# sinhvt3421/scann--material

Measured on AMD Instinct MI355X. Metric: QM9 molecules/s forward, higher is better.
Workload: dtype f32 (projections: split-fp16 hi/lo operands, 3 v_mfma_f32_32x32x16_f16 per product, fp32 accumulate; everything else fp32)

## Files before the change

include/scann_hip.h:

```cpp
#ifndef SCANN_HIP_H
#define SCANN_HIP_H

#include <stdint.h>

#ifdef __cplusplus
extern "C" {
#endif

#define SCANN_ABI_VERSION 1

typedef enum scann_status {
  SCANN_OK = 0,
  SCANN_ERR_INVALID = -1,
  SCANN_ERR_UNSUPPORTED = -2,
  SCANN_ERR_NO_DEVICE = -3,
  SCANN_ERR_HIP = -4,
  SCANN_ERR_WEIGHTS = -5,
  SCANN_ERR_OOM = -6,
  SCANN_ERR_RANGE = -7
} scann_status;

typedef struct scann_config {
  int32_t n_atoms;
  int32_t embedding_dim;
  int32_t local_dim;
  int32_t num_head;
  int32_t n_attention;
  int32_t global_dim;
  int32_t dense_out;
  int32_t n_gauss;
  float gaussian_d;
  int32_t g_update;
  int32_t use_attn_norm;
  int32_t use_ga_norm;
  int32_t use_ring;
  int32_t feature_cgcnn;
  int32_t relu_out;
} scann_config_t;

typedef struct scann_tensor_desc {
  const char* name;
  int64_t offset;
  int64_t numel;
} scann_tensor_desc_t;

typedef struct scann_batch {
  int32_t n_struct;
  int32_t n_atom;
  int32_t n_edge;
  const int32_t* atomic;
  const int32_t* mol_offset;
  const int32_t* edge_offset;
  const int32_t* edge_col;
  const float* edge_dist;
  const float* edge_weight;
  const float* ring;
  const float* cgcnn;
} scann_batch_t;

typedef struct scann_handle scann_handle_t;
typedef struct scann_dbatch scann_dbatch_t;

typedef struct scann_profile {
  float ms_basis;
  float ms_atom;
  float ms_edge;
  float ms_readout;
  float ms_total;
  int32_t n_edge_launch;
  int32_t n_atom_launch;
  int32_t reserved;
} scann_profile_t;

int scann_abi_version(void);
int scann_device_count(void);

int scann_create(const scann_config_t* cfg, int device_id, scann_handle_t** out);
void scann_destroy(scann_handle_t* h);
const char* scann_last_error(const scann_handle_t* h);

int scann_weight_count(const scann_handle_t* h);
int scann_weight_name(const scann_handle_t* h, int index, const char** name, int64_t* rows, int64_t* cols);

int scann_load_weights(scann_handle_t* h, const float* blob, const scann_tensor_desc_t* manifest, int n);

int scann_forward(scann_handle_t* h, const scann_batch_t* batch, float* y_out, float* ga_attn_out);

int scann_forward_padded(scann_handle_t* h, int32_t B, int32_t M, int32_t N, const int32_t* atomic,
                         const uint8_t* atom_mask, const int32_t* neighbors, const uint8_t* neighbor_mask,
                         const float* neighbor_weight, const float* neighbor_distance, float* y_out, float* ga_out);

int scann_batch_upload(scann_handle_t* h, const scann_batch_t* batch, scann_dbatch_t** out);
int scann_upload_padded(scann_handle_t* h, int32_t B, int32_t M, int32_t N, const int32_t* atomic, const void* atom_mask,
                        int32_t atom_mask_size, const int32_t* neighbors, const void* neighbor_mask, int32_t neighbor_mask_size,
                        const float* neighbor_weight, const float* neighbor_distance, scann_dbatch_t** out, int32_t* n_atom_out,
                        int32_t* n_edge_out);
int scann_batch_read_csr(scann_handle_t* h, scann_dbatch_t* db, int32_t* atomic, int32_t* mol_offset, int32_t* edge_offset,
                         int32_t* edge_col, float* edge_dist, float* edge_weight);
void scann_batch_free(scann_handle_t* h, scann_dbatch_t* db);
void scann_batch_release(scann_handle_t* h, scann_dbatch_t* db);
int scann_forward_resident(scann_handle_t* h, scann_dbatch_t* db, int stream_slot);
int scann_batch_download(scann_handle_t* h, scann_dbatch_t* db, float* y_out, float* ga_attn_out);
int scann_batch_info(scann_handle_t* h, const scann_dbatch_t* db, int32_t* out8);
int scann_sync(scann_handle_t* h);
int scann_device_memory(scann_handle_t* h, int64_t* free_bytes, int64_t* total_bytes);
int64_t scann_exact_reruns(const scann_handle_t* h);
int scann_weights_exact(const scann_handle_t* h);
int scann_num_streams(const scann_handle_t* h);

#define SCANN_OUT_LOCAL_ATTENTION 0
#define SCANN_OUT_AFTER_LC 1
#define SCANN_OUT_BF_PROPERTY 2
int scann_set_outputs(scann_handle_t* h, uint64_t attn_layers, int32_t flags);
int64_t scann_output_read(scann_handle_t* h, scann_dbatch_t* db, int32_t what, int32_t layer, float* out, int64_t cap);

int scann_forward_profile(scann_handle_t* h, scann_dbatch_t* db, scann_profile_t* prof);

int scann_edge_timing(scann_handle_t* h, int every);
int scann_edge_timing_read(scann_handle_t* h, double* avg_us, int64_t* n_launches, double* avg_edges);

int scann_set_debug(scann_handle_t* h, int on);
int scann_debug_read(scann_handle_t* h, scann_dbatch_t* db, int what, int layer, float* out);
int64_t scann_train_debug_read(scann_handle_t* h, scann_dbatch_t* db, const char* name, float* out, int64_t cap);

int scann_debug_stamps(scann_handle_t* h, scann_dbatch_t* db, uint64_t* out, int max_tiles);

int64_t scann_param_count(const scann_handle_t* h);
int scann_train_begin(scann_handle_t* h);
int scann_train_forward(scann_handle_t* h, scann_dbatch_t* db, const float* targets, float dropout, uint64_t seed, double* sse_out);
int scann_train_backward(scann_handle_t* h, scann_dbatch_t* db, double sse_global, int64_t count_global);
int scann_set_attention_dropout(scann_handle_t* h, float p);
int scann_set_deterministic(scann_handle_t* h, int on);
int scann_zero_grads(scann_handle_t* h);
int scann_allreduce_grads(scann_handle_t* h);
int scann_allreduce_sse(scann_handle_t* h, double* sse, int64_t* count);
int scann_adam_step(scann_handle_t* h, float lr_t, float beta1, float beta2, float eps, float l2);
int scann_train_step(scann_handle_t* h, scann_dbatch_t* db, const float* targets, float dropout, uint64_t seed, float lr_t, float beta1,
                     float beta2, float eps, float l2, double* sse_out, int64_t* count_out);
int scann_train_step_begin(scann_handle_t* h, scann_dbatch_t* db, const float* targets, float dropout, uint64_t seed, float lr_t, float beta1,
                           float beta2, float eps, float l2);
int scann_train_step_end(scann_handle_t* h, double* sse_out, int64_t* count_out, double* abs_err_out );
int scann_get_grads(scann_handle_t* h, float* out);
int scann_get_weights(scann_handle_t* h, float* out);

int scann_input_grads(scann_handle_t* h, scann_dbatch_t* db, float* y, float* d_distance, float* d_weight,
                      float* d_ring, float* d_cgcnn);

int scann_predict_mc(scann_handle_t* h, scann_dbatch_t* db, int32_t n_samples, uint64_t seed, const uint64_t* keys, float p_drop, float p_attn,
                     float* y_mean, float* y_std, float* ga_mean, float* ga_std, float* y_samples);
double scann_mc_drop_scale(uint64_t seed, int32_t t, uint64_t key, uint32_t tag, uint64_t idx, float p);

#define SCANN_ABLATE_LEAVE_ONE_OUT 0
#define SCANN_ABLATE_DELETION 1
#define SCANN_ABLATE_INSERTION 2
#define SCANN_ABLATE_MAX_ATOMS 960
int scann_ablate_pooling(scann_handle_t* h, scann_dbatch_t* db, int32_t mode, float* y, float* ga, float* y_abl, int32_t* order);

int scann_shapley(scann_handle_t* h, scann_dbatch_t* db, int32_t n_perm, uint64_t seed, const uint64_t* keys, const int32_t* perms_in,
                  float* y, float* ga, double* shapley, double* stderr_out, double* baseline, double* full, float* values, int32_t* perms_out);
int scann_shapley_profile(scann_handle_t* h, scann_dbatch_t* db, int32_t n_perm, uint64_t seed, const uint64_t* keys, float* ms);
void scann_shapley_permutation(uint64_t seed, uint64_t key, int32_t p, int32_t n, int32_t* out);
int scann_shapley_reduce_host(const float* values, const int32_t* perms, const int32_t* mol_offset, int32_t n_struct, int32_t n_perm,
                              const double* baseline, double* shapley, double* stderr_out, double* full);

#define SCANN_ROLLOUT_MAX_ATOMS 960
int64_t scann_rollout_floats(scann_handle_t* h, const scann_dbatch_t* db);
int scann_attention_rollout(scann_handle_t* h, scann_dbatch_t* db, float residual, int32_t head, int32_t depth, float* y, float* ga,
                            float* attribution, float* rollout);

#define SCANN_KNN_MAX_K 32
typedef struct scann_index scann_index_t;
int scann_index_create(scann_handle_t* h, int32_t dim, scann_index_t** out);
void scann_index_free(scann_handle_t* h, scann_index_t* idx);
int64_t scann_index_size(const scann_index_t* idx);
int scann_index_add(scann_handle_t* h, scann_index_t* idx, const float* rows, int64_t n, const int64_t* ids, const int32_t* atoms);
int scann_index_read(scann_handle_t* h, scann_index_t* idx, int64_t first, int64_t n, float* rows, int64_t* ids, int32_t* atoms);
int scann_index_query(scann_handle_t* h, scann_index_t* idx, const float* q, int64_t nq, const int64_t* query_ids, int32_t k, float* dist2,
                      int64_t* ids, int32_t* atoms, int32_t* pos);
int scann_index_add_batch(scann_handle_t* h, scann_index_t* idx, scann_dbatch_t* db, int32_t level, const int64_t* ids);
// ... 110 lines not shown
                       int64_t* sums);
int scann_peaks_host(const float* rows, int64_t n, int64_t dim, float gamma, int64_t* sums, int32_t* parent, float* delta2);

#define SCANN_MST_MAX_ROWS 262144
int scann_index_mst(scann_handle_t* h, scann_index_t* pool, const float* core2 , int64_t* n_edges,
                    int32_t* a , int32_t* b, float* w, int32_t* rounds );
int scann_mst_host(const float* rows, int64_t n, int64_t dim, const float* core2, int64_t* n_edges, int32_t* a, int32_t* b, float* w);
int scann_mst_last_rounds(int32_t cap, int32_t* components, double* seconds, int64_t* skipped, int64_t* tiles);

int scann_index_silhouette(scann_handle_t* h, scann_index_t* pool, const int32_t* labels , int32_t C,
                           const int32_t* qpos , int64_t nq, int32_t squared, int32_t shift,
                           int64_t* counts , double* a , double* b , int32_t* other ,
                           int64_t* sums );
int scann_silhouette_host(const float* rows, int64_t n, int64_t dim, const int32_t* labels, int32_t C, const int32_t* qpos, int64_t nq,
                          int32_t squared, int32_t shift, int32_t threads, int64_t* counts, double* a, double* b, int32_t* other,
                          int64_t* sums);

#define SCANN_RANKS_MAX_PROBES 32
#define SCANN_RANKS_SLICE 262144
int scann_index_ranks(scann_handle_t* h, scann_index_t* pool,
                      const int32_t* qpos , int64_t nq,
                      const int32_t* probe , int32_t m,
                      int32_t* rank , float* dist2 );
int scann_ranks_host(const float* rows, int64_t n, int64_t dim, const int32_t* qpos, int64_t nq, const int32_t* probe, int32_t m,
                     int32_t threads, int32_t* rank, float* dist2);

int scann_index_partition(scann_handle_t* h, scann_index_t* idx, int32_t cells, int32_t max_iter, int64_t* info );
int scann_index_partition_args(const scann_index_t* idx, int32_t* cells, int32_t* max_iter);
int scann_index_cells_read(scann_handle_t* h, scann_index_t* idx, int64_t* info , float* centres, int32_t* perm, int32_t* first_tile,
                           float* lo, float* hi);
int scann_index_search_stats(const scann_index_t* idx, int64_t* out );
int scann_index_query_rows(scann_handle_t* h, scann_index_t* idx, int64_t first, int64_t n, int32_t k, float* dist2, int64_t* ids,
                           int32_t* atoms, int32_t* pos);
int64_t scann_cells_capacity(int64_t n, int32_t cells);
int scann_cells_host(const float* rows, int64_t n, int64_t dim, int32_t cells, int32_t max_iter, int64_t* info, float* centres, int32_t* perm,
                     int32_t* first_tile, float* lo, float* hi);
double scann_cell_bound(float D, float lo, float hi);

#define SCANN_WITHIN_MAX_CAP ((int64_t)1 << 30)
int scann_index_within(scann_handle_t* h, scann_index_t* idx, const float* q, int64_t nq, const int64_t* query_ids, float radius2, int64_t cap,
                       int64_t* counts , int64_t* total, float* dist2, int32_t* pos, int64_t* ids, int32_t* atoms );
int scann_index_within_rows(scann_handle_t* h, scann_index_t* idx, int64_t first, int64_t n, int32_t upper, float radius2, int64_t cap,
                            int64_t* counts, int64_t* total, float* dist2, int32_t* pos, int64_t* ids, int32_t* atoms);
int scann_index_within_batch(scann_handle_t* h, scann_index_t* idx, scann_dbatch_t* db, int32_t level, const int64_t* query_ids, float radius2,
                             int64_t cap, float* y, float* ga, int64_t* counts, int64_t* total, float* dist2, int32_t* pos, int64_t* ids,
                             int32_t* atoms);
int scann_within_host(const float* rows, int64_t n, int64_t dim, const int64_t* row_ids, const float* q, int64_t nq, const int64_t* query_ids,
                      const int32_t* query_pos, int32_t upper, float radius2, int64_t cap, int64_t* counts, int64_t* total, float* dist2,
                      int32_t* pos);

int scann_comm_unique_id(char* out128);
int scann_comm_init(scann_handle_t* h, const char* id128, int rank, int world);
int scann_comm_ranks(scann_handle_t* h);
int scann_broadcast_weights(scann_handle_t* h, int root);

int scann_models_load(scann_handle_t* h, int32_t n_models, const float* const* blobs, const scann_tensor_desc_t* const* manifests,
                      const int32_t* n_tensors, const int32_t* relu_out);
int scann_models_count(const scann_handle_t* h);
int scann_forward_models(scann_handle_t* h, scann_dbatch_t* db, int stream_slot);
int scann_models_download(scann_handle_t* h, scann_dbatch_t* db, float* y, float* ga);

const char* scann_pack_last_error(void);
int scann_pack_padded(int32_t B, int32_t M, int32_t N, const int32_t* atomic, const float* cgcnn,
                      const uint8_t* atom_mask, const int32_t* neighbors, const uint8_t* neighbor_mask,
                      const float* neighbor_weight, const float* neighbor_distance, const float* ring,
                      int32_t* out_atomic, float* out_cgcnn, float* out_ring, int32_t* out_mol_offset,
                      int32_t* out_edge_offset, int32_t* out_edge_col, float* out_edge_dist,
                      float* out_edge_weight, int32_t* out_row_of, int32_t* n_atom, int32_t* n_edge);
int scann_slice_count(const int64_t* ds_mol_offset, const int64_t* ds_edge_offset, const int64_t* sel, int32_t n_sel,
                      int64_t n_struct_total, int64_t* n_atom, int64_t* n_edge);
int scann_slice_batch(const int64_t* ds_mol_offset, const int64_t* ds_edge_offset, const int32_t* ds_atomic,
                      const float* ds_ring, const int32_t* ds_edge_local, const float* ds_edge_dist,
                      const float* ds_edge_weight, const int64_t* sel, int32_t n_sel, int64_t n_struct_total,
                      int32_t* out_atomic, float* out_ring, int32_t* out_mol_offset, int32_t* out_edge_offset,
                      int32_t* out_edge_col, float* out_edge_dist, float* out_edge_weight);
int scann_count_padded(int32_t B, int32_t M, int32_t N, const void* atom_mask, int32_t atom_mask_size, const void* neighbor_mask,
                       int32_t neighbor_mask_size, int32_t* out_mol_offset, int32_t* out_edge_offset, int32_t* out_row_of,
                       int32_t* n_atom, int32_t* n_edge);
int scann_host_copy(void* dst, const void* src, int64_t bytes);
int scann_plan_tiles(const scann_batch_t* batch, int32_t tile_rows, int32_t tile_atoms, int32_t allow_chunks, int32_t cap,
                     int32_t* tiles_out, int32_t* part_out, int32_t* n_tiles, int32_t* n_slots);
int scann_plan_tiles_filled(const scann_batch_t* batch, int32_t tile_rows, int32_t tile_atoms, int32_t cap, int32_t* atom_row_out,
                            int32_t* tile_offset_out, int32_t* tiles_out, int32_t* n_tiles);
int scann_batch_tile_plan(scann_handle_t* h, const scann_dbatch_t* batch, int32_t* out2);

#ifdef __cplusplus
}
#endif
#endif
```

scann--material_amd/csrc/scann_batch.cpp:

```cpp
#include "scann_runtime.h"

namespace {

struct PaddedSrc {
  int32_t M, N;
  const int32_t *atomic, *neighbors;
  const void* neighbor_mask;
  int32_t mask_size;
  const float *weight, *dist;
  const int32_t* row_of;
  const int32_t *d_atomic = nullptr, *d_neighbors = nullptr;
  const void* d_mask = nullptr;
  const float *d_weight = nullptr, *d_dist = nullptr;
};

}

static inline void par_memcpy(void* dst, const void* src, size_t bytes) { (void)scann_host_copy(dst, src, (int64_t)bytes); }

static int upload_impl(scann_handle_t* h, const scann_batch_t* b, scann_dbatch_t** out, bool scratch, const PaddedSrc* pad = nullptr) {
  if (!h || !b || !out) return fail(h, SCANN_ERR_INVALID, "scann_batch_upload: null argument");
  *out = nullptr;
  const int32_t B = b->n_struct, A = b->n_atom, E = b->n_edge;
  if (B <= 0 || A <= 0 || E < 0) return fail(h, SCANN_ERR_INVALID, "scann_batch_upload: empty batch");
  if (!b->mol_offset || !b->edge_offset ||
      (!pad && ((!b->atomic && !h->cfg.feature_cgcnn) || (E > 0 && (!b->edge_col || !b->edge_dist || !b->edge_weight)))))
    return fail(h, SCANN_ERR_INVALID, "scann_batch_upload: null array");
  if (pad && (h->cfg.feature_cgcnn || h->cfg.use_ring || h->t_master))
    return fail(h, SCANN_ERR_UNSUPPORTED, "scann_upload_padded: atomic feature without ring, inference handles (a training handle needs the edges on the host)");
  if (b->mol_offset[0] != 0 || b->mol_offset[B] != A || b->edge_offset[0] != 0 || b->edge_offset[A] != E)
    return fail(h, SCANN_ERR_INVALID, "scann_batch_upload: offsets do not cover the batch");
  int32_t max_atoms = 0;
  for (int s = 0; s < B; ++s) {
    const int32_t n = b->mol_offset[s + 1] - b->mol_offset[s];
    if (n <= 0) return fail(h, SCANN_ERR_INVALID, "scann_batch_upload: structure without atoms");
    max_atoms = std::max(max_atoms, n);
  }
  if ((size_t)max_atoms * 5 * sizeof(float) > 60000) return fail(h, SCANN_ERR_UNSUPPORTED, "scann_batch_upload: structure too large");
  if ((uint64_t)std::max(A, E) * D * 4 >= (1ull << 32))
    return fail(h, SCANN_ERR_UNSUPPORTED, "scann_batch_upload: more than 8,388,607 atoms or edges in one batch; split it");
  if (pad) {
  } else if (!h->cfg.feature_cgcnn) {
    for (int a = 0; a < A; ++a)
      if (b->atomic[a] < 0 || b->atomic[a] >= h->cfg.n_atoms)
        return fail(h, SCANN_ERR_INVALID, "scann_batch_upload: atomic number outside the embedding table (n_atoms)");
  } else if (!b->cgcnn) {
    return fail(h, SCANN_ERR_INVALID, "scann_batch_upload: feature=cgcnn needs batch.cgcnn [n_atom,92]");
  }
  if (h->cfg.use_ring && !b->ring) return fail(h, SCANN_ERR_INVALID, "scann_batch_upload: use_ring needs batch.ring [n_atom,2]");
  std::vector<int32_t> edge_row;
  std::vector<EdgeTile> tiles;
  std::vector<int32_t> tile_part, big_tab;
  int32_t n_slot = 0, max_degree = 0;
  int tile_rows = TE_MAX;
  {
    std::string err;
    const bool small = E > 0 && E <= 32 * 1024;
    int r = plan_tiles(b->mol_offset, B, b->edge_offset, pad ? nullptr : b->edge_col, A, E, small ? 32 : TE_MAX, h->tile_atoms, true, tiles,
                       tile_part, big_tab, edge_row, &tile_rows, &max_degree, &n_slot, err, false);
    if (r) return fail(h, r, "scann_batch_upload: " + err);
    if (small && max_degree > 32) {
      r = plan_tiles(b->mol_offset, B, b->edge_offset, pad ? nullptr : b->edge_col, A, E, TE_MAX, h->tile_atoms, true, tiles, tile_part, big_tab, edge_row,
                     &tile_rows, &max_degree, &n_slot, err, false);
      if (r) return fail(h, r, "scann_batch_upload: " + err);
    }
  }
  const int32_t n_big = (int32_t)big_tab.size() / 3;
  const bool tile_side = h->cfg.g_update && !h->generic && E > 0;
  const size_t n_ftile = tiles.size();
  HIPCHK(h, hipSetDevice(h->device));
  scann_dbatch* db = nullptr;
  if (scratch) {
    if (!h->sc_db) h->sc_db = new scann_dbatch();
    db = h->sc_db;
    if (db->dbg_c || db->stamps) (void)hipStreamSynchronize(h->streams[0]);
    cached_free(db->dbg_c);
    cached_free(db->dbg_g);
    cached_free(db->dbg_ctx);
    cached_free(db->fill_block);
    if (db->stamps) (void)hipFree(db->stamps);
    char* const gen_ws = db->gen_ws;
    const size_t gen_ws_bytes = db->gen_ws_bytes;
    char* const out_block = db->out_block;
    const size_t out_cap = db->out_cap;
    char* const mc_ws = db->mc_ws;
    const size_t mc_bytes = db->mc_bytes;
    char* const set_ws = db->set_ws;
    const size_t set_bytes = db->set_bytes;
    *db = scann_dbatch();
    db->set_ws = set_ws; db->set_bytes = set_bytes;
    db->gen_ws = gen_ws; db->gen_ws_bytes = gen_ws_bytes;
    db->out_block = out_block; db->out_cap = out_cap;
    db->mc_ws = mc_ws; db->mc_bytes = mc_bytes;
    db->owns_arena = false;
  } else {
    db = new scann_dbatch();
  }
  db->n_struct = B; db->n_atom = A; db->n_edge = E; db->n_tile = (int32_t)tiles.size(); db->max_atoms = max_atoms; db->tile_rows = tile_rows; db->max_degree = max_degree; db->tile_atoms = h->tile_atoms; db->n_big = n_big; db->n_slot = n_slot;
  size_t off = 0;
  auto take = [&](size_t bytes) { const size_t o = off; off = align_up(off + bytes); return o; };
  const size_t o_atomic = take((size_t)A * 4), o_mol = take((size_t)(B + 1) * 4), o_eoff = take((size_t)(A + 1) * 4);
  const size_t o_col = take((size_t)E * 4), o_row = take((size_t)E * 4), o_dist = take((size_t)E * 4), o_wgt = take((size_t)E * 4);
  const size_t o_tiles = take(tiles.size() * sizeof(EdgeTile));
  const size_t o_tpart = take(n_big ? tiles.size() * 4 : 0), o_big = take((size_t)n_big * 3 * 4);
  const size_t o_inoff = take((size_t)(A + 1) * 4), o_inedge = take((size_t)E * 4);
  const size_t o_ring = take(h->cfg.use_ring ? (size_t)A * 2 * 4 : 0), o_cg = take(h->cfg.feature_cgcnn ? (size_t)A * 92 * 4 : 0);
  const size_t BM = pad ? (size_t)B * pad->M : 0, BMN = pad ? BM * pad->N : 0;
  const bool pre = pad && pad->d_atomic;
  const size_t o_prow = take(BM * 4), o_pat = take(pre ? 0 : BM * 4), o_pnbr = take(pre ? 0 : BMN * 4);
  const size_t o_pmask = take(pad && !pre ? BMN * pad->mask_size : 0), o_pw = take(pre ? 0 : BMN * 4), o_pd = take(pre ? 0 : BMN * 4);
  const size_t in_bytes = off;
  const size_t rowA = (size_t)A * D * 4, rowE = (size_t)std::max(E, 1) * D * 4;
  const size_t o_geom = take(h->cfg.g_update ? rowE + D * 4 : 0);
  const size_t o_gd = take(h->cfg.g_update ? 0 : (size_t)std::max(E, 1) * NG * 4);
  const size_t o_c0 = take((h->cfg.use_ring || h->cfg.feature_cgcnn) ? rowA : 0);
  const size_t o_c = take(rowA), o_ctx = take(rowA), o_P1 = take(rowA), o_P3 = take(rowA), o_q = take(rowA);
  const size_t o_gq = take(rowA), o_gk = take(rowA), o_ga = take((size_t)A * 4), o_y = take((size_t)B * 4);
  const size_t o_pflag = take(pad ? 4 : 0);
  const size_t o_pbuf = take((size_t)n_slot * 3 * D * 4);
  const size_t slot_bytes = tile_side ? n_ftile * TQ * 4 : 0;
  const size_t o_tatom = take(slot_bytes), o_te0 = take(slot_bytes), o_tsp = take(h->cfg.feature_cgcnn ? 0 : slot_bytes);
  hipError_t e = hipSuccess;
  scann_handle::Stage* stage = nullptr;
  char* img_ptr = nullptr;
  if (scratch) {
    if (off > h->sc_cap) {
      if (h->sc_arena) { (void)hipStreamSynchronize(h->streams[0]); (void)hipFree(h->sc_arena); h->sc_arena = nullptr; h->sc_cap = 0; }
      const size_t want = off + off / 2;
      e = hipMalloc((void**)&h->sc_arena, want);
      if (e == hipSuccess) h->sc_cap = want;
    }
    if (e == hipSuccess && in_bytes > h->sc_host_cap) {
      if (h->sc_host) { (void)hipStreamSynchronize(h->streams[0]); (void)hipHostFree(h->sc_host); h->sc_host = nullptr; h->sc_host_cap = 0; }
      const size_t want = in_bytes + in_bytes / 2;
      e = hipHostMalloc((void**)&h->sc_host, want, hipHostMallocDefault);
      if (e == hipSuccess) h->sc_host_cap = want;
    }
    db->arena = h->sc_arena;
    img_ptr = h->sc_host;
  } else {
    e = cached_malloc((void**)&db->arena, off);
    if (e == hipSuccess && !h->copy_stream) e = hipStreamCreateWithFlags(&h->copy_stream, hipStreamNonBlocking);
    if (e == hipSuccess) {
      stage = &h->stage[h->stage_next++ % scann_handle::N_STAGE];
      if (stage->used) (void)hipEventSynchronize(stage->ev);
      if (!stage->ev) e = hipEventCreateWithFlags(&stage->ev, hipEventDisableTiming);
      if (e == hipSuccess && in_bytes > stage->cap) {
        if (stage->p) (void)hipHostFree(stage->p);
        stage->p = nullptr; stage->cap = 0;
        const size_t want = in_bytes + in_bytes / 4;
        e = hipHostMalloc((void**)&stage->p, want, hipHostMallocDefault);
        if (e == hipSuccess) stage->cap = want;
      }
      img_ptr = stage->p;
    }
  }
  if (e != hipSuccess) {
    if (!scratch) {
      if (db->arena) cached_free(db->arena);
      delete db;
    }
    return fail(h, e == hipErrorOutOfMemory ? SCANN_ERR_OOM : SCANN_ERR_HIP, std::string("hipMalloc(batch arena): ") + hipGetErrorString(e));
  }
  struct ImgView { char* p; char* data() const { return p; } } img{img_ptr};
  if (b->atomic && !pad) memcpy(img.data() + o_atomic, b->atomic, (size_t)A * 4);
  if (pad) memcpy(img.data() + o_prow, pad->row_of, BM * 4);
  if (pad && !pre) {
    memcpy(img.data() + o_pat, pad->atomic, BM * 4);
    par_memcpy(img.data() + o_pnbr, pad->neighbors, BMN * 4);
    par_memcpy(img.data() + o_pmask, pad->neighbor_mask, BMN * pad->mask_size);
    par_memcpy(img.data() + o_pw, pad->weight, BMN * 4);
    par_memcpy(img.data() + o_pd, pad->dist, BMN * 4);
  }
  if (h->cfg.use_ring) memcpy(img.data() + o_ring, b->ring, (size_t)A * 2 * 4);
  if (h->cfg.feature_cgcnn) memcpy(img.data() + o_cg, b->cgcnn, (size_t)A * 92 * 4);
  memcpy(img.data() + o_mol, b->mol_offset, (size_t)(B + 1) * 4);
  memcpy(img.data() + o_eoff, b->edge_offset, (size_t)(A + 1) * 4);
  if (E > 0 && !pad) {
    memcpy(img.data() + o_col, b->edge_col, (size_t)E * 4);
    memcpy(img.data() + o_dist, b->edge_dist, (size_t)E * 4);
    memcpy(img.data() + o_wgt, b->edge_weight, (size_t)E * 4);
  }
  memcpy(img.data() + o_tiles, tiles.data(), tiles.size() * sizeof(EdgeTile));
  const bool want_rev = h->t_master != nullptr;
  if (want_rev) {
    int32_t* in_off = reinterpret_cast<int32_t*>(img.data() + o_inoff);
    int32_t* in_edge = reinterpret_cast<int32_t*>(img.data() + o_inedge);
    memset(in_off, 0, (size_t)(A + 1) * 4);
    for (int e = 0; e < E; ++e) ++in_off[b->edge_col[e] + 1];
    for (int a = 0; a < A; ++a) in_off[a + 1] += in_off[a];
    std::vector<int32_t> fill(in_off, in_off + A);
    for (int e = 0; e < E; ++e) in_edge[fill[b->edge_col[e]]++] = e;
  }
  if (n_big) {
    memcpy(img.data() + o_tpart, tile_part.data(), tiles.size() * 4);
    memcpy(img.data() + o_big, big_tab.data(), (size_t)n_big * 3 * 4);
  }
  int32_t* const d_eoff = (int32_t*)(db->arena + o_eoff);
  int32_t* const d_erow = (int32_t*)(db->arena + o_row);
  PackPaddedArgs pa{};
  if (pad) {
    char* a0 = db->arena;
    pa.B = B; pa.M = pad->M; pa.N = pad->N; pa.n_species = h->cfg.n_atoms;
    pa.row_of = (const int32_t*)(a0 + o_prow); pa.edge_offset = d_eoff; pa.atomic = pre ? pad->d_atomic : (const int32_t*)(a0 + o_pat);
    pa.neighbors = pre ? pad->d_neighbors : (const int32_t*)(a0 + o_pnbr); pa.neighbor_mask = pre ? pad->d_mask : a0 + o_pmask;
    pa.mask_size = pad->mask_size;
    pa.weight = pre ? pad->d_weight : (const float*)(a0 + o_pw); pa.dist = pre ? pad->d_dist : (const float*)(a0 + o_pd);
    pa.out_atomic = (int32_t*)(a0 + o_atomic); pa.out_col = (int32_t*)(a0 + o_col);
    pa.out_dist = (float*)(a0 + o_dist); pa.out_weight = (float*)(a0 + o_wgt);
    pa.flag = (int32_t*)(a0 + o_pflag);
  }
  TileOrderArgs ta{};
  if (tile_side) {
    char* a0 = db->arena;
    ta.tiles = (const EdgeTile*)(a0 + o_tiles); ta.n_tile = (int32_t)n_ftile; ta.n_atom = A;
    ta.edge_offset = d_eoff; ta.atomic = h->cfg.feature_cgcnn ? nullptr : (const int32_t*)(a0 + o_atomic);
    ta.tile_atom = (int32_t*)(a0 + o_tatom); ta.tile_edge0 = (int32_t*)(a0 + o_te0); ta.tile_species = (int32_t*)(a0 + o_tsp);
  }
  if (scratch) {
    if (e == hipSuccess) e = hipMemcpyAsync(db->arena, img.data(), in_bytes, hipMemcpyHostToDevice, h->streams[0]);
    if (e == hipSuccess && (E > 0 || pad)) launch_edge_row(d_eoff, E > 0 ? A : 0, d_erow, h->streams[0], pad ? pa.flag : nullptr);
    if (e == hipSuccess && pad) launch_pack_padded(pa, h->streams[0]);
    if (e == hipSuccess && tile_side) launch_tile_order(ta, h->streams[0]);
  } else {
    if (e == hipSuccess) e = hipMemcpyAsync(db->arena, img.data(), in_bytes, hipMemcpyHostToDevice, h->copy_stream);
    if (e == hipSuccess && (E > 0 || pad)) launch_edge_row(d_eoff, E > 0 ? A : 0, d_erow, h->copy_stream, pad ? pa.flag : nullptr);
    if (e == hipSuccess && pad) launch_pack_padded(pa, h->copy_stream);
    if (e == hipSuccess && tile_side) launch_tile_order(ta, h->copy_stream);
    if (e == hipSuccess) e = hipEventRecord(stage->ev, h->copy_stream);
    if (e == hipSuccess) stage->used = true;
    if (e == hipSuccess) e = hipEventCreateWithFlags(&db->upload_ev, hipEventDisableTiming);
    if (e == hipSuccess) e = hipEventRecord(db->upload_ev, h->copy_stream);
  }
  if (e != hipSuccess) {
    if (!scratch) {
      (void)hipStreamSynchronize(h->copy_stream);
      if (db->upload_ev) (void)hipEventDestroy(db->upload_ev);
      cached_free(db->arena);
      delete db;
    }
    return fail(h, SCANN_ERR_HIP, std::string("hipMemcpy(batch inputs): ") + hipGetErrorString(e));
  }
  char* a0 = db->arena;
  db->atomic = (int32_t*)(a0 + o_atomic); db->mol_offset = (int32_t*)(a0 + o_mol); db->edge_offset = (int32_t*)(a0 + o_eoff);
  db->edge_col = (int32_t*)(a0 + o_col); db->edge_row = (int32_t*)(a0 + o_row);
  db->dist = (float*)(a0 + o_dist); db->weight = (float*)(a0 + o_wgt); db->tiles = (EdgeTile*)(a0 + o_tiles);
  db->in_off = (int32_t*)(a0 + o_inoff); db->in_edge = (int32_t*)(a0 + o_inedge);
  db->has_rev = want_rev;
  db->n_ftile = (int32_t)n_ftile;
  db->f_tiles = db->tiles; db->t_offset = db->edge_offset; db->t_col = db->edge_col; db->t_row = db->edge_row;
  db->t_dist = db->dist; db->t_weight = db->weight;
  if (tile_side) {
    db->tile_atom = (int32_t*)(a0 + o_tatom); db->tile_edge0 = (int32_t*)(a0 + o_te0);
    db->tile_species = h->cfg.feature_cgcnn ? nullptr : (int32_t*)(a0 + o_tsp);
  }
  db->ring = (float*)(a0 + o_ring); db->cgcnn = (float*)(a0 + o_cg); db->c0 = (float*)(a0 + o_c0);
  db->geom = (float*)(a0 + o_geom); db->gd = (float*)(a0 + o_gd);
  db->c = (float*)(a0 + o_c); db->ctx = (float*)(a0 + o_ctx); db->P1 = (float*)(a0 + o_P1); db->P3 = (float*)(a0 + o_P3);
  db->q = (float*)(a0 + o_q); db->gq = (float*)(a0 + o_gq); db->gk = (float*)(a0 + o_gk);
  db->ga = (float*)(a0 + o_ga); db->y = (float*)(a0 + o_y);
  db->pack_flag = pad ? (int32_t*)(a0 + o_pflag) : nullptr;
  if (n_big) {
    db->tile_part = (int32_t*)(a0 + o_tpart); db->big_tab = (int32_t*)(a0 + o_big); db->part_buf = (float*)(a0 + o_pbuf);
  }
  *out = db;
  return SCANN_OK;
}

static int fetch_results(scann_handle_t* h, scann_dbatch_t* db, hipStream_t s, float* y_out, float* ga_attn_out) {
  const char* src = reinterpret_cast<const char*>(ga_attn_out ? db->ga : db->y);
  const size_t y_off = (size_t)(reinterpret_cast<const char*>(db->y) - src);
  const size_t f_off = db->pack_flag ? (size_t)(reinterpret_cast<const char*>(db->pack_flag) - src) : 0;
  const size_t bytes = db->pack_flag ? f_off + 4 : y_off + (size_t)db->n_struct * 4;
  scann_handle::DlStage& st = h->dl_stage[db->last_slot];
  if (st.cap < bytes) {
    if (st.p) {
      HIPCHK(h, hipStreamSynchronize(s));
      (void)hipHostFree(st.p);
      st.p = nullptr;
      st.cap = 0;
    }
    const size_t cap = std::max<size_t>(bytes + bytes / 2, (size_t)1 << 16);
    HIPCHK(h, hipHostMalloc((void**)&st.p, cap, hipHostMallocDefault));
    st.cap = cap;
  }
  HIPCHK(h, hipMemcpyAsync(st.p, src, bytes, hipMemcpyDeviceToHost, s));
  HIPCHK(h, hipStreamSynchronize(s));
  if (db->pack_flag) {
    const int32_t bad = *reinterpret_cast<const int32_t*>(st.p + f_off);
    if (bad & 1) return fail(h, SCANN_ERR_INVALID, "scann_batch_download: an unmasked neighbour slot points at a padded atom (or outside the structure)");
    if (bad & 2) return fail(h, SCANN_ERR_INVALID, "scann_batch_download: atomic number outside the embedding table (n_atoms)");
  }
  if (y_out) memcpy(y_out, st.p + y_off, (size_t)db->n_struct * 4);
  if (ga_attn_out) memcpy(ga_attn_out, st.p, (size_t)db->n_atom * 4);
  return SCANN_OK;
}

namespace scann {

void free_batch(scann_dbatch* db) {
  if (db->arena && db->owns_arena) cached_free(db->arena);
  cached_free(db->gen_ws);
  cached_free(db->out_block);
  cached_free(db->mc_ws);
  cached_free(db->set_ws);
  cached_free(db->dbg_c);
  cached_free(db->dbg_g);
  cached_free(db->dbg_ctx);
  cached_free(db->fill_block);
  if (db->stamps) (void)hipFree(db->stamps);
  if (db->upload_ev) (void)hipEventDestroy(db->upload_ev);
  delete db;
}

int check_pack_flag(scann_handle_t* h, scann_dbatch_t* db, const char* who) {
  if (!db->pack_flag) return SCANN_OK;
  int32_t bad = 0;
  HIPCHK(h, hipMemcpy(&bad, db->pack_flag, 4, hipMemcpyDeviceToHost));
  if (bad & 1) return fail(h, SCANN_ERR_INVALID, std::string(who) + ": an unmasked neighbour slot points at a padded atom (or outside the structure)");
  if (bad & 2) return fail(h, SCANN_ERR_INVALID, std::string(who) + ": atomic number outside the embedding table (n_atoms)");
  return SCANN_OK;
}

int ensure_tile_fill(scann_handle_t* h, scann_dbatch_t* db, hipStream_t s) {
  if (db->fill_tried) return SCANN_OK;
  db->fill_tried = true;
  if (!h->tile_fill || !db->tile_atom || db->n_big > 0 || db->n_tile <= 1) return SCANN_OK;
  const int32_t B = db->n_struct, A = db->n_atom, E = db->n_edge;
  std::vector<int32_t> mol((size_t)B + 1), eoff((size_t)A + 1), atom_row, tile_offset;
  std::vector<EdgeTile> ftiles;
  if (db->upload_ev && !db->upload_done) HIPCHK(h, hipEventSynchronize(db->upload_ev));
  else if (!db->upload_ev) HIPCHK(h, hipStreamSynchronize(h->streams[0]));
  HIPCHK(h, hipMemcpy(mol.data(), db->mol_offset, mol.size() * 4, hipMemcpyDeviceToHost));
  HIPCHK(h, hipMemcpy(eoff.data(), db->edge_offset, eoff.size() * 4, hipMemcpyDeviceToHost));
  const std::vector<EdgeTile> contiguous((size_t)db->n_tile);
  if (!plan_tiles_filled(mol.data(), B, eoff.data(), A, db->tile_rows, db->tile_atoms, contiguous, db->n_big, atom_row, tile_offset, ftiles))
    return SCANN_OK;
// ... 8 lines not shown
  memcpy(img.data() + o_arow, atom_row.data(), (size_t)A * 4);
  memcpy(img.data() + o_toff, tile_offset.data(), (size_t)(A + 1) * 4);
  memcpy(img.data() + o_ftiles, ftiles.data(), nt * sizeof(EdgeTile));
  char* blk = nullptr;
  if (cached_malloc((void**)&blk, off) != hipSuccess) return SCANN_OK;
  hipError_t e = hipMemcpy(blk, img.data(), in_bytes, hipMemcpyHostToDevice);
  TileOrderArgs ta{};
  ta.tiles = (const EdgeTile*)(blk + o_ftiles); ta.n_tile = (int32_t)nt; ta.n_atom = A;
  ta.atom_row = (const int32_t*)(blk + o_arow); ta.tile_offset = (const int32_t*)(blk + o_toff);
  ta.edge_offset = db->edge_offset; ta.atomic = db->tile_species ? db->atomic : nullptr;
  ta.col = db->edge_col; ta.dist = db->dist; ta.weight = db->weight;
  ta.tile_atom = (int32_t*)(blk + o_tatom); ta.tile_edge0 = (int32_t*)(blk + o_te0); ta.tile_species = (int32_t*)(blk + o_tsp);
  ta.out_col = (int32_t*)(blk + o_tcol); ta.out_row = (int32_t*)(blk + o_trow);
  ta.out_dist = (float*)(blk + o_tdist); ta.out_weight = (float*)(blk + o_twgt);
  if (e == hipSuccess) {
    launch_tile_order(ta, s);
    e = hipStreamSynchronize(s);
  }
  if (e != hipSuccess) {
    cached_free(blk);
    return fail(h, SCANN_ERR_HIP, std::string("filled tile plan: ") + hipGetErrorString(e));
  }
  db->fill_block = blk;
  db->filled = true; db->n_ftile = (int32_t)nt;
  db->f_tiles = (EdgeTile*)(blk + o_ftiles); db->t_offset = (int32_t*)(blk + o_toff);
  db->t_col = ta.out_col; db->t_row = ta.out_row; db->t_dist = ta.out_dist; db->t_weight = ta.out_weight;
  db->tile_atom = ta.tile_atom; db->tile_edge0 = ta.tile_edge0;
  if (db->tile_species) db->tile_species = ta.tile_species;
  return SCANN_OK;
}

int rerun_if_out_of_range(scann_handle_t* h, scann_dbatch_t* db, hipStream_t s, bool* rerun) {
  *rerun = false;
  if (!h->range_flag || h->strict_range || db->kept) return SCANN_OK;
  const int32_t code = *reinterpret_cast<volatile int32_t*>(h->range_flag + db->last_slot);
  const int site = code >> 8;
  if (!code || site < 1 || site > 4) return SCANN_OK;
  h->range_flag[db->last_slot] = 0;
  FwdOpts o;
  o.exact = true;
  o.out_layers = db->out_layers;
  o.out_flags = db->out_flags;
  const int r = run_forward(h, db, s, o);
  if (r) return r;
  h->exact_reruns++;
  *rerun = true;
  HIPCHK(h, hipStreamSynchronize(s));
  return SCANN_OK;
}

static int download(scann_handle_t* h, scann_dbatch_t* db, float* y_out, float* ga_attn_out) {
  hipStream_t s = h->streams[db->last_slot];
  const int rf = fetch_results(h, db, s, y_out, ga_attn_out);
  if (rf) return rf;
  bool rerun = false;
  if (const int r = rerun_if_out_of_range(h, db, s, &rerun)) return r;
  if (rerun) {
    const int rf3 = fetch_results(h, db, s, y_out, ga_attn_out);
    if (rf3) return rf3;
  }
  db->idle = true;
  db->fwd_pending = false;
  return check_range(h, "scann_batch_download", db->last_slot);
}

int forward_and_download(scann_handle_t* h, scann_dbatch_t* db, uint64_t layers, int32_t flags, float* y, float* ga) {
  HIPCHK(h, hipSetDevice(h->device));
  if (const int r = run_forward(h, db, h->streams[db->last_slot], selected_opts(h, layers, flags))) return r;
  return download(h, db, y, ga);
}

int read_mol_offset(scann_handle_t* h, const scann_dbatch_t* db, std::vector<int32_t>& mol) {
  mol.assign((size_t)db->n_struct + 1, 0);
  if (db->upload_ev && !db->upload_done) HIPCHK(h, hipEventSynchronize(db->upload_ev));
  if (db->n_struct > 0) HIPCHK(h, hipMemcpy(mol.data(), db->mol_offset, mol.size() * 4, hipMemcpyDeviceToHost));
  return SCANN_OK;
}

}

extern "C" {

int scann_batch_upload(scann_handle_t* h, const scann_batch_t* b, scann_dbatch_t** out) { return upload_impl(h, b, out, false); }

int scann_upload_padded(scann_handle_t* h, int32_t B, int32_t M, int32_t N, const int32_t* atomic, const void* atom_mask,
                        int32_t atom_mask_size, const int32_t* neighbors, const void* neighbor_mask, int32_t neighbor_mask_size,
                        const float* neighbor_weight, const float* neighbor_distance, scann_dbatch_t** out, int32_t* n_atom_out,
                        int32_t* n_edge_out) {
  if (!h || !out || B <= 0 || M <= 0 || N < 0 || !atomic || !atom_mask || (N > 0 && (!neighbors || !neighbor_mask || !neighbor_weight || !neighbor_distance)))
    return fail(h, SCANN_ERR_INVALID, "scann_upload_padded: bad argument");
  *out = nullptr;
  const size_t BM = (size_t)B * M;
  std::vector<int32_t> row_of(BM), mol((size_t)B + 1), eoff(BM + 1);
  int32_t na = 0, ne = 0;
  if (scann_count_padded(B, M, N, atom_mask, atom_mask_size, neighbor_mask, neighbor_mask_size, mol.data(), eoff.data(), row_of.data(), &na, &ne))
    return fail(h, SCANN_ERR_INVALID, std::string("scann_upload_padded: ") + scann_pack_last_error());
  scann_batch_t pb{};
  pb.n_struct = B; pb.n_atom = na; pb.n_edge = ne; pb.mol_offset = mol.data(); pb.edge_offset = eoff.data();
  const PaddedSrc src{M, N, atomic, neighbors, neighbor_mask, neighbor_mask_size, neighbor_weight, neighbor_distance, row_of.data()};
  const int r = upload_impl(h, &pb, out, false, &src);
  if (r) return r;
  if (n_atom_out) *n_atom_out = na;
  if (n_edge_out) *n_edge_out = ne;
  return SCANN_OK;
}

void scann_batch_free(scann_handle_t* h, scann_dbatch_t* db) {
  if (!db) return;
  if (h) (void)hipSetDevice(h->device);
  if (h) (void)hipDeviceSynchronize();
  free_batch(db);
}

void scann_batch_release(scann_handle_t* h, scann_dbatch_t* db) {
  if (!db) return;
  const bool step_done = db->busy_ev && hipEventQuery(db->busy_ev) == hipSuccess;
  if (!h || !(step_done || (db->idle && db->set_busy < 0))) {
    scann_batch_free(h, db);
    return;
  }
  (void)hipSetDevice(h->device);
  free_batch(db);
}

int scann_batch_info(scann_handle_t* h, const scann_dbatch_t* db, int32_t* out8) {
  if (!h || !db || !out8) return fail(h, SCANN_ERR_INVALID, "scann_batch_info: null argument");
  out8[0] = db->n_struct; out8[1] = db->n_atom; out8[2] = db->n_edge; out8[3] = db->n_big;
  out8[4] = db->n_slot; out8[5] = db->max_degree; out8[6] = db->n_tile; out8[7] = db->tile_rows;
  return SCANN_OK;
}

int scann_batch_tile_plan(scann_handle_t* h, const scann_dbatch_t* db, int32_t* out2) {
  if (!h || !db || !out2) return fail(h, SCANN_ERR_INVALID, "scann_batch_tile_plan: null argument");
  out2[0] = db->filled ? 1 : 0;
  out2[1] = db->tile_atom ? db->n_ftile : db->n_tile;
  return SCANN_OK;
}

int scann_batch_download(scann_handle_t* h, scann_dbatch_t* db, float* y_out, float* ga_attn_out) {
  if (!h || !db || !y_out) return fail(h, SCANN_ERR_INVALID, "scann_batch_download: null argument");
  HIPCHK(h, hipSetDevice(h->device));
  return download(h, db, y_out, ga_attn_out);
}

int scann_device_memory(scann_handle_t* h, int64_t* free_bytes, int64_t* total_bytes) {
  if (!h || !free_bytes || !total_bytes) return fail(h, SCANN_ERR_INVALID, "scann_device_memory: null argument");
  HIPCHK(h, hipSetDevice(h->device));
  size_t f = 0, t = 0;
  HIPCHK(h, hipMemGetInfo(&f, &t));
  *free_bytes = (int64_t)f;
  *total_bytes = (int64_t)t;
  return SCANN_OK;
}

int scann_forward(scann_handle_t* h, const scann_batch_t* batch, float* y_out, float* ga_attn_out) {
  scann_dbatch_t* db = nullptr;
  int r = upload_impl(h, batch, &db, true);
  if (r) return r;
  r = scann_forward_resident(h, db, 0);
  if (!r) r = scann_batch_download(h, db, y_out, ga_attn_out);
  return r;
}

int scann_forward_padded(scann_handle_t* h, int32_t B, int32_t M, int32_t N, const int32_t* atomic, const uint8_t* atom_mask,
                         const int32_t* neighbors, const uint8_t* neighbor_mask, const float* neighbor_weight,
                         const float* neighbor_distance, float* y_out, float* ga_out) {
  if (!h || B <= 0 || M <= 0 || N < 0 || !atomic || !atom_mask || !y_out || (N > 0 && (!neighbors || !neighbor_mask || !neighbor_weight || !neighbor_distance)))
    return fail(h, SCANN_ERR_INVALID, "scann_forward_padded: bad argument");
  if (h->cfg.use_ring || h->cfg.feature_cgcnn) return fail(h, SCANN_ERR_UNSUPPORTED, "scann_forward_padded: atomic feature without ring only");
  const size_t BM = (size_t)B * M;
  scann_handle::PadScratch& ps = h->pad_scratch;
  auto grow_i = [](std::vector<int32_t>& v, size_t n) { if (v.size() < n) v.resize(n + n / 4); };
  auto grow_f = [](std::vector<float>& v, size_t n) { if (v.size() < n) v.resize(n + n / 4); };
  grow_i(ps.gidx, BM); grow_i(ps.mol, (size_t)B + 1); grow_i(ps.eoff, BM + 1);
  std::vector<int32_t>&gidx = ps.gidx, &mol = ps.mol, &eoff = ps.eoff;
  int32_t na = 0, ne = 0;
  const bool device_pack = !h->t_master;
  scann_batch_t pb{};
  std::vector<float>& ga_packed = ps.ga;
  int r;
  if (device_pack) {
    HIPCHK(h, hipSetDevice(h->device));
    const size_t BMN = BM * (size_t)N;
    const size_t p_at = 0, p_nbr = align_up(BM * 4), p_mask = p_nbr + align_up(BMN * 4), p_w = p_mask + align_up(BMN), p_d = p_w + align_up(BMN * 4);
    const size_t p_bytes = p_d + align_up(BMN * 4);
    if (p_bytes > h->pp_cap) {
      HIPCHK(h, hipStreamSynchronize(h->streams[0]));
// ... 67 lines not shown
```

scann--material_amd/csrc/scann_internal.h:

```cpp
#pragma once
#include <hip/hip_runtime.h>
#include <stdint.h>

#include <string>
#include <vector>

namespace scann {

constexpr int D = 128;
constexpr int NHEAD = 8;
constexpr int HDIM = D / NHEAD;
constexpr int NG = 20;
constexpr int LDS_STRIDE = 132;
constexpr int TE_MAX = 64;
constexpr int TA = 64;
constexpr int TQ = 24;
constexpr int WPACK = D * D;
constexpr float WSCALE = 256.f;
constexpr float WMAX = 65504.f / WSCALE;

__host__ __device__ inline float drop_scale(unsigned long long seed, unsigned tag, size_t idx, float p) {
  unsigned long long z = seed + 0x9E3779B97F4A7C15ull * (idx + 1) + ((unsigned long long)tag << 48);
  z = (z ^ (z >> 30)) * 0xBF58476D1CE4E5B9ull;
  z = (z ^ (z >> 27)) * 0x94D049BB133111EBull;
// ... 253 lines not shown
void launch_gen_dense_dw(const GenDwArgs& a, hipStream_t s);
int gen_ln_chunks(int rows);
void launch_gen_layernorm_bwd(const float* X, const float* res, const float* gamma, const float* dY, int rows, int N, float* dX, float* stats,
                              float* part, float* dgamma, float* dbeta, hipStream_t s);
void launch_gen_attn_bwd(const float* q, const float* K, const int32_t* edge_offset, int n_atom, int d, int H, int max_degree, const float* dctx,
                         float drop_p, unsigned drop_tag, unsigned long long drop_seed, float* dq, float* dK, hipStream_t s);
void launch_gen_pool_bwd(const int32_t* mol_offset, int n_struct, int max_atoms, const float* gq, const float* gk, int dg, int use_ga_norm,
                         const float* drep, float* dgq, float* dgk, hipStream_t s);
void launch_gen_edge_to_atom(const int32_t* edge_offset, const int32_t* in_off, const int32_t* in_edge, const float* S_out, const float* S_in,
                             const float* P_a, const float* P_b, const float* acc, int n_atom, int d, float* out, hipStream_t s);
void launch_gen_table_grad(const int32_t* atomic, int n_atom, const float* dV, int emb, int n_species, float* part, float* dTable, hipStream_t s);

struct ReadoutArgs {
  const int32_t* mol_offset;
  int32_t n_struct;
  int32_t max_atoms;
  const float *gq, *gk;
  int32_t use_ga_norm, relu_out;
  HeadParams p;
  float* ga_attn;
  float* y;
  float* bf_out;
  int32_t n_member;
  int64_t m_w, m_a, m_g, m_y;
};
void launch_readout(const ReadoutArgs& a, hipStream_t s);

struct AblateArgs {
  const int32_t* mol_offset;
  int32_t n_struct, max_atoms;
  const float *gq, *gk;
  int32_t dg, dout;
  int32_t use_ga_norm, relu_out, mode;
  const float *Wb, *bb, *wo, *bo;
  const float* ga_attn;
  float* y_abl;
  int32_t* order;
};
size_t ablate_lds_bytes(int max_atoms, int dg);
hipError_t launch_ablate(const AblateArgs& a, bool mfma, hipStream_t s);

struct ShapleyArgs {
  const int32_t* mol_offset;
  int32_t n_struct, n_atom, max_atoms, n_perm;
  const float *gq, *gk;
  int32_t dg, dout;
  int32_t use_ga_norm, relu_out;
  const float *Wb, *bb, *wo, *bo;
  unsigned long long seed;
  const unsigned long long* keys;
  const int32_t* perms_in;
  const int64_t* pair_offset;
  float* pair;
  float* values;
  int32_t* perms;
  double *shapley, *stderr_out;
  double *baseline, *full;
};
constexpr int SHAPLEY_PCHUNK = 4;
hipError_t launch_shapley(const ShapleyArgs& a, bool mfma, hipStream_t s, hipEvent_t* ev = nullptr);
void shapley_reduce_host(const float* values, const int32_t* perms, const int32_t* mol_offset, int n_struct, int n_perm, const double* baseline,
                         double* shapley, double* stderr_out, double* full);

struct RolloutArgs {
  const int32_t *mol_offset, *edge_offset, *edge_col;
  int32_t n_struct, n_edge, max_atoms;
  int32_t num_head, head, depth;
  float residual;
  const float* attn;
  const float* ga;
  float* abar;
  float* attribution;
  float* rollout;
  const int64_t* roll_offset;
};
int rollout_slab(int max_atoms);
size_t rollout_lds_bytes(int max_atoms);
hipError_t launch_rollout(const RolloutArgs& a, hipStream_t s);

int plan_tiles(const int32_t* mol_offset, int32_t B, const int32_t* edge_offset, const int32_t* edge_col, int32_t A, int32_t E,
               int tile_rows_req, int tile_atoms, bool allow_chunks, std::vector<EdgeTile>& tiles, std::vector<int32_t>& tile_part,
               std::vector<int32_t>& big_tab, std::vector<int32_t>& edge_row, int* tile_rows_out, int32_t* max_degree,
               int32_t* n_slot, std::string& err, bool fill_edge_row = true);
bool plan_tiles_filled(const int32_t* mol_offset, int32_t B, const int32_t* edge_offset, int32_t A, int rows, int tile_atoms,
                       const std::vector<EdgeTile>& contiguous, int32_t n_big, std::vector<int32_t>& atom_row,
                       std::vector<int32_t>& tile_offset, std::vector<EdgeTile>& tiles);
struct TileOrderArgs {
  const EdgeTile* tiles;
  int32_t n_tile, n_atom;
  const int32_t* atom_row;
  const int32_t* tile_offset;
  const int32_t* edge_offset;
  const int32_t* atomic;
  const int32_t* col;
  const float *dist, *weight;
  int32_t *tile_atom, *tile_edge0, *tile_species;
  int32_t *out_col, *out_row;
  float *out_dist, *out_weight;
};
void launch_tile_order(const TileOrderArgs& a, hipStream_t s);
void launch_edge_row(const int32_t* edge_offset, int n_atom, int32_t* edge_row, hipStream_t s, int32_t* zero_word = nullptr);

struct PackPaddedArgs {
  int32_t B, M, N, n_species;
  const int32_t* row_of;
  const int32_t* edge_offset;
  const int32_t* atomic;
  const int32_t* neighbors;
  const void* neighbor_mask;
  int32_t mask_size;
  const float *weight, *dist;
  int32_t* out_atomic;
  int32_t* out_col;
  float *out_dist, *out_weight;
  int32_t* flag;
};
void launch_pack_padded(const PackPaddedArgs& a, hipStream_t s);

void pack_weight(const float* W, int ld, float* Wp);
void pack_weight_f16(const float* W, int ld, int k_real, int ks, uint16_t* out);

}
```

scann--material_amd/csrc/scann_pack.cpp:

```cpp
#include <cstdint>
#include <cstdio>
#include <cstring>
#include <string>

#include <algorithm>
#include <thread>
#include <vector>

#include "../../include/scann_hip.h"
#include "scann_internal.h"

namespace {
thread_local std::string t_pack_error;
int pack_fail(const char* msg) {
  t_pack_error = msg;
  return SCANN_ERR_INVALID;
}

template <class Fn>
void fan_out(int n, Fn&& fn) {
  std::vector<std::thread> th;
  int t = 1;
  try {
    th.reserve((size_t)std::max(0, n - 1));
// ... 20 lines not shown

namespace scann {

static void tile_range(const int32_t* edge_offset, int32_t a0, int32_t a1, int want, int tile_atoms, bool allow_chunks,
                       std::vector<EdgeTile>& tiles, std::vector<int32_t>& tile_part, std::vector<int32_t>& big_tab, int32_t& n_slot) {
  EdgeTile cur{a0, a0, edge_offset[a0], edge_offset[a0]};
  for (int a = a0; a < a1; ++a) {
    const int32_t e0 = edge_offset[a], e1 = edge_offset[a + 1];
    if (allow_chunks && e1 - e0 > want) {
      if (a > cur.atom_begin) {
        cur.atom_end = a;
        cur.edge_end = e0;
        tiles.push_back(cur);
        tile_part.push_back(-1);
      }
      big_tab.push_back(a); big_tab.push_back(n_slot); big_tab.push_back((e1 - e0 + want - 1) / want);
      for (int c0 = e0; c0 < e1; c0 += want) {
        tiles.push_back(EdgeTile{a, a + 1, c0, std::min(c0 + want, e1)});
        tile_part.push_back(n_slot++);
      }
      cur = EdgeTile{a + 1, a + 1, e1, e1};
      continue;
    }
    if ((e1 - cur.edge_begin) > want || (a - cur.atom_begin) >= tile_atoms) {
      cur.atom_end = a;
      cur.edge_end = e0;
      tiles.push_back(cur);
      tile_part.push_back(-1);
      cur = EdgeTile{a, a, e0, e0};
    }
  }
  if (cur.atom_begin < a1) {
    cur.atom_end = a1;
    cur.edge_end = edge_offset[a1];
    tiles.push_back(cur);
    tile_part.push_back(-1);
  }
}

int plan_tiles(const int32_t* mol_offset, int32_t B, const int32_t* edge_offset, const int32_t* edge_col, int32_t A, int32_t E,
               int tile_rows_req, int tile_atoms, bool allow_chunks, std::vector<EdgeTile>& tiles, std::vector<int32_t>& tile_part,
               std::vector<int32_t>& big_tab, std::vector<int32_t>& edge_row, int* tile_rows_out, int32_t* max_degree,
               int32_t* n_slot_out, std::string& err, bool fill_edge_row) {
  int32_t n_slot = 0, maxdeg = 0, mindeg = 0;
  for (int a = 0; a < A; ++a) {
    const int32_t deg = edge_offset[a + 1] - edge_offset[a];
    maxdeg = std::max(maxdeg, deg);
    mindeg = std::min(mindeg, deg);
  }
  if (mindeg < 0) { err = "edge_offset not monotone"; return SCANN_ERR_INVALID; }
  if (maxdeg > TE_MAX && !allow_chunks) {
    err = "an atom has more than 64 neighbours (edge-tile limit of the selected edge kernel; edge_kernel_lean, the default on "
          "the g_update path, has none)";
    return SCANN_ERR_UNSUPPORTED;
  }
  for (int s = 0; s < B && edge_col; ++s) {
    const int32_t a0 = mol_offset[s], a1 = mol_offset[s + 1];
    int32_t mn = a0, mx = a0;
    for (int e = edge_offset[a0]; e < edge_offset[a1]; ++e) {
      mn = std::min(mn, edge_col[e]);
      mx = std::max(mx, edge_col[e]);
    }
    if (mn < a0 || mx >= a1) { err = "neighbour index outside its structure"; return SCANN_ERR_INVALID; }
  }
  if (fill_edge_row) {
    edge_row.resize((size_t)E);
    for (int a = 0; a < A; ++a)
      for (int e = edge_offset[a]; e < edge_offset[a + 1]; ++e) edge_row[(size_t)e] = a;
  }
  int tile_rows = tile_rows_req;
  if (maxdeg > tile_rows && !allow_chunks) tile_rows = TE_MAX;
  tiles.clear(); tile_part.clear(); big_tab.clear(); n_slot = 0;
  tile_range(edge_offset, 0, A, tile_rows, tile_atoms, allow_chunks, tiles, tile_part, big_tab, n_slot);
  if (tiles.empty()) {
    tiles.push_back(EdgeTile{0, A, 0, E});
    tile_part.push_back(-1);
  }
  *tile_rows_out = tile_rows;
  *max_degree = maxdeg;
  *n_slot_out = n_slot;
  return SCANN_OK;
}

bool plan_tiles_filled(const int32_t* mol_offset, int32_t B, const int32_t* edge_offset, int32_t A, int rows, int tile_atoms,
                       const std::vector<EdgeTile>& contiguous, int32_t n_big, std::vector<int32_t>& atom_row,
                       std::vector<int32_t>& tile_offset, std::vector<EdgeTile>& tiles) {
  const auto identity = [&]() {
    atom_row.resize((size_t)A);
    for (int a = 0; a < A; ++a) atom_row[(size_t)a] = a;
    tile_offset.assign(edge_offset, edge_offset + A + 1);
    tiles = contiguous;
    return false;
  };
  if (n_big > 0 || rows > 64 || rows <= 0 || tile_atoms <= 0 || contiguous.size() <= 1) return identity();
  atom_row.resize((size_t)A);
  tile_offset.resize((size_t)A + 1);
  tiles.clear();
  tiles.reserve(contiguous.size());
  int32_t* const out_row = atom_row.data();
  int32_t* const out_off = tile_offset.data();
  out_off[0] = 0;
  std::vector<int32_t> order_buf;
  int32_t cnt[66] = {}, head[66], tail[66], fill[66];
  EdgeTile cur{0, 0, 0, 0};
  int32_t k = 0, e = 0;
  for (int s = 0; s < B; ++s) {
    const int32_t a0 = mol_offset[s], a1 = mol_offset[s + 1];
    int maxd = 0;
    for (int a = a0; a < a1; ++a) {
      const int d = edge_offset[a + 1] - edge_offset[a];
      if (d > rows) return identity();
      ++cnt[d];
      maxd = std::max(maxd, d);
    }
    uint64_t lo = 0;
    bool top = false;
    for (int d = 0, pos = 0; d <= maxd; ++d) {
      head[d] = fill[d] = pos;
      if (cnt[d]) { if (d < 64) lo |= 1ull << d; else top = true; }
      pos += cnt[d];
      tail[d] = pos;
      cnt[d] = 0;
    }
    if (order_buf.size() < (size_t)(a1 - a0)) order_buf.resize((size_t)(a1 - a0) * 2);
    int32_t* const order = order_buf.data();
    for (int a = a0; a < a1; ++a) order[fill[edge_offset[a + 1] - edge_offset[a]]++] = a;
    for (int left = a1 - a0; left > 0; --left) {
      const int room = (k - cur.atom_begin) >= tile_atoms ? -1 : rows - (e - cur.edge_begin);
      int d = -1;
      if (room >= 64 && top) d = 64;
      else if (room >= 0) {
        const uint64_t fit = room >= 63 ? lo : lo & ((2ull << room) - 1);
        if (fit) d = 63 - __builtin_clzll(fit);
      }
      if (d < 0) {
        cur.atom_end = k; cur.edge_end = e;
        tiles.push_back(cur);
        cur = EdgeTile{k, k, e, e};
        d = top ? 64 : 63 - __builtin_clzll(lo);
      }
      const int32_t a = order[head[d]++];
      if (head[d] == tail[d]) { if (d < 64) lo &= ~(1ull << d); else top = false; }
      out_row[k++] = a;
      e += d;
      out_off[k] = e;
    }
  }
  cur.atom_end = k; cur.edge_end = e;
  tiles.push_back(cur);
  if (tiles.size() >= contiguous.size()) return identity();
  return true;
}


}

extern "C" {

const char* scann_pack_last_error(void) { return t_pack_error.c_str(); }

int scann_pack_padded(int32_t B, int32_t M, int32_t N, const int32_t* atomic, const float* cgcnn,
                      const uint8_t* atom_mask, const int32_t* neighbors, const uint8_t* neighbor_mask,
                      const float* neighbor_weight, const float* neighbor_distance, const float* ring,
                      int32_t* out_atomic, float* out_cgcnn, float* out_ring, int32_t* out_mol_offset,
                      int32_t* out_edge_offset, int32_t* out_edge_col, float* out_edge_dist,
                      float* out_edge_weight, int32_t* out_row_of, int32_t* n_atom, int32_t* n_edge) {
  if (B < 0 || M < 0 || N < 0 || !atom_mask ||
      (N > 0 && (!neighbors || !neighbor_mask || !neighbor_weight || !neighbor_distance)) || !out_mol_offset || !out_edge_offset || !out_edge_col || !out_edge_dist ||
      !out_edge_weight || !out_row_of || !n_atom || !n_edge)
    return pack_fail("scann_pack_padded: null argument or negative shape");
  if ((atomic && !out_atomic) || (cgcnn && !out_cgcnn) || (ring && !out_ring))
    return pack_fail("scann_pack_padded: an input is given without its output array");
  const int n_thr = pack_threads(B);
  std::vector<int64_t> cnt_a((size_t)n_thr + 1, 0), cnt_e((size_t)n_thr + 1, 0);
  std::vector<const char*> err((size_t)n_thr, nullptr);
  fan_out(n_thr, [&](int t) {
    const auto [b0, b1] = pack_range(B, t, n_thr);
    int64_t na_t = 0, ne_t = 0;
    for (int32_t b = b0; b < b1; ++b) {
      const uint8_t* am = atom_mask + (int64_t)b * M;
      int64_t here = 0;
      for (int32_t a = 0; a < M; ++a) {
        if (!am[a]) continue;
        ++here;
        const uint8_t* nm = neighbor_mask + ((int64_t)b * M + a) * N;
        for (int32_t n = 0; n < N; ++n) ne_t += nm[n] != 0;
      }
      if (here == 0) { err[t] = "a structure in the batch has no atoms"; return; }
      na_t += here;
    }
    cnt_a[t + 1] = na_t;
    cnt_e[t + 1] = ne_t;
  });
  for (int t = 0; t < n_thr; ++t) {
    if (err[t]) return pack_fail(err[t]);
    cnt_a[t + 1] += cnt_a[t];
    cnt_e[t + 1] += cnt_e[t];
  }
  const int64_t na = cnt_a[n_thr], ne = cnt_e[n_thr];
  if (na > INT32_MAX) return pack_fail("batch too large for int32 atom rows");
  if (ne > INT32_MAX) return pack_fail("batch too large for int32 edge rows");
  out_mol_offset[0] = 0;
  out_edge_offset[0] = 0;
  fan_out(n_thr, [&](int t) {
    const auto [b0, b1] = pack_range(B, t, n_thr);
    int64_t row = cnt_a[t], e = cnt_e[t];
    for (int32_t b = b0; b < b1; ++b) {
      const uint8_t* am = atom_mask + (int64_t)b * M;
      int32_t* ro = out_row_of + (int64_t)b * M;
      int64_t r = row;
      for (int32_t a = 0; a < M; ++a) ro[a] = am[a] ? (int32_t)r++ : -1;
      for (int32_t a = 0; a < M; ++a) {
        if (ro[a] < 0) continue;
        const int64_t base = ((int64_t)b * M + a) * N;
        for (int32_t n = 0; n < N; ++n) {
          if (!neighbor_mask[base + n]) continue;
          const int32_t tgt = neighbors[base + n];
          if (tgt < 0 || tgt >= M || ro[tgt] < 0) { err[t] = "an unmasked neighbour slot points at a padded atom"; return; }
          out_edge_col[e] = ro[tgt];
          out_edge_dist[e] = neighbor_distance[base + n];
          out_edge_weight[e] = neighbor_weight[base + n];
          ++e;
        }
        if (atomic) out_atomic[row] = atomic[(int64_t)b * M + a];
        if (cgcnn) memcpy(out_cgcnn + row * 92, cgcnn + ((int64_t)b * M + a) * 92, 92 * sizeof(float));
        if (ring) memcpy(out_ring + row * 2, ring + ((int64_t)b * M + a) * 2, 2 * sizeof(float));
        out_edge_offset[++row] = (int32_t)e;
      }
      out_mol_offset[b + 1] = (int32_t)row;
    }
  });
  for (int t = 0; t < n_thr; ++t)
    if (err[t]) return pack_fail(err[t]);
  *n_atom = (int32_t)na;
  *n_edge = (int32_t)ne;
  return SCANN_OK;
}
// ... 96 lines not shown
    const int64_t s = sel[i];
    if (s < 0 || s >= n_struct_total) return pack_fail("scann_slice_count: structure index out of range");
    const int64_t a0 = ds_mol_offset[s], a1 = ds_mol_offset[s + 1];
    na += a1 - a0;
    ne += ds_edge_offset[a1] - ds_edge_offset[a0];
  }
  *n_atom = na;
  *n_edge = ne;
  return SCANN_OK;
}

int scann_slice_batch(const int64_t* ds_mol_offset, const int64_t* ds_edge_offset, const int32_t* ds_atomic,
                      const float* ds_ring, const int32_t* ds_edge_local, const float* ds_edge_dist,
                      const float* ds_edge_weight, const int64_t* sel, int32_t n_sel, int64_t n_struct_total,
                      int32_t* out_atomic, float* out_ring, int32_t* out_mol_offset, int32_t* out_edge_offset,
                      int32_t* out_edge_col, float* out_edge_dist, float* out_edge_weight) {
  if (!ds_mol_offset || !ds_edge_offset || !ds_atomic || !ds_edge_local || !ds_edge_dist || !ds_edge_weight ||
      (!sel && n_sel) || n_sel < 0 || !out_atomic || !out_mol_offset || !out_edge_offset || !out_edge_col ||
      !out_edge_dist || !out_edge_weight || (ds_ring && !out_ring))
    return pack_fail("scann_slice_batch: null argument");
  int64_t na = 0, ne = 0;
  out_mol_offset[0] = 0;
  out_edge_offset[0] = 0;
  for (int32_t i = 0; i < n_sel; ++i) {
    const int64_t s = sel[i];
    if (s < 0 || s >= n_struct_total) return pack_fail("scann_slice_batch: structure index out of range");
    const int64_t a0 = ds_mol_offset[s], a1 = ds_mol_offset[s + 1];
    const int64_t e0 = ds_edge_offset[a0], e1 = ds_edge_offset[a1];
    const int64_t cnt = a1 - a0, ecnt = e1 - e0;
    if (cnt <= 0) return pack_fail("a structure in the batch has no atoms");
    if (na + cnt > INT32_MAX || ne + ecnt > INT32_MAX) return pack_fail("batch too large for int32 rows");
    memcpy(out_atomic + na, ds_atomic + a0, cnt * sizeof(int32_t));
    if (ds_ring) memcpy(out_ring + na * 2, ds_ring + a0 * 2, cnt * 2 * sizeof(float));
    const int64_t shift = ne - e0;
    for (int64_t a = 0; a < cnt; ++a) out_edge_offset[na + a + 1] = (int32_t)(ds_edge_offset[a0 + a + 1] + shift);
    const int32_t base = (int32_t)na;
    for (int64_t e = 0; e < ecnt; ++e) {
      const int32_t l = ds_edge_local[e0 + e];
      if (l < 0 || l >= cnt) return pack_fail("a neighbour index lies outside its structure");
      out_edge_col[ne + e] = base + l;
    }
    memcpy(out_edge_dist + ne, ds_edge_dist + e0, ecnt * sizeof(float));
    memcpy(out_edge_weight + ne, ds_edge_weight + e0, ecnt * sizeof(float));
    na += cnt;
    ne += ecnt;
    out_mol_offset[i + 1] = (int32_t)na;
  }
  return SCANN_OK;
}

int scann_plan_tiles(const scann_batch_t* b, int32_t tile_rows, int32_t tile_atoms, int32_t allow_chunks, int32_t cap,
                     int32_t* tiles_out, int32_t* part_out, int32_t* n_tiles, int32_t* n_slots) {
  if (!b || !n_tiles || !n_slots || !b->mol_offset || !b->edge_offset || (b->n_edge > 0 && !b->edge_col) || b->n_struct <= 0 ||
      b->n_atom <= 0 || b->n_edge < 0 || (tile_rows != 32 && tile_rows != 64) || tile_atoms <= 0 || tile_atoms > 32)
    return pack_fail("scann_plan_tiles: bad argument");
  if (b->mol_offset[0] != 0 || b->mol_offset[b->n_struct] != b->n_atom || b->edge_offset[0] != 0 || b->edge_offset[b->n_atom] != b->n_edge)
    return pack_fail("scann_plan_tiles: offsets do not cover the batch");
  for (int s = 0; s < b->n_struct; ++s)
    if (b->mol_offset[s + 1] <= b->mol_offset[s]) return pack_fail("scann_plan_tiles: structure without atoms");
  std::vector<scann::EdgeTile> tiles;
  std::vector<int32_t> part, big, row;
  int rows = 0;
  int32_t maxdeg = 0, nslot = 0;
  std::string err;
  const int r = scann::plan_tiles(b->mol_offset, b->n_struct, b->edge_offset, b->edge_col, b->n_atom, b->n_edge, tile_rows, tile_atoms,
                                  allow_chunks != 0, tiles, part, big, row, &rows, &maxdeg, &nslot, err);
  if (r) {
    t_pack_error = "scann_plan_tiles: " + err;
    return r;
  }
  *n_tiles = (int32_t)tiles.size();
  *n_slots = nslot;
  if ((int32_t)tiles.size() > cap || !tiles_out || !part_out) return tiles_out ? pack_fail("scann_plan_tiles: output capacity too small") : SCANN_OK;
  for (size_t i = 0; i < tiles.size(); ++i) {
    tiles_out[4 * i] = tiles[i].atom_begin; tiles_out[4 * i + 1] = tiles[i].atom_end;
    tiles_out[4 * i + 2] = tiles[i].edge_begin; tiles_out[4 * i + 3] = tiles[i].edge_end;
    part_out[i] = part[i];
  }
  return rows;
}

int scann_plan_tiles_filled(const scann_batch_t* b, int32_t tile_rows, int32_t tile_atoms, int32_t cap, int32_t* atom_row_out,
                            int32_t* tile_offset_out, int32_t* tiles_out, int32_t* n_tiles) {
  if (!b || !n_tiles || !atom_row_out || !tile_offset_out || !tiles_out || !b->mol_offset || !b->edge_offset || b->n_struct <= 0 ||
      b->n_atom <= 0 || b->n_edge < 0 || (tile_rows != 32 && tile_rows != 64) || tile_atoms <= 0 || tile_atoms > 32)
    return pack_fail("scann_plan_tiles_filled: bad argument");
  if (b->mol_offset[0] != 0 || b->mol_offset[b->n_struct] != b->n_atom || b->edge_offset[0] != 0 || b->edge_offset[b->n_atom] != b->n_edge)
    return pack_fail("scann_plan_tiles_filled: offsets do not cover the batch");
  for (int s = 0; s < b->n_struct; ++s)
    if (b->mol_offset[s + 1] <= b->mol_offset[s]) return pack_fail("scann_plan_tiles_filled: structure without atoms");
  std::vector<scann::EdgeTile> contiguous, tiles;
  std::vector<int32_t> part, big, row, atom_row, tile_offset;
  int rows = 0;
  int32_t maxdeg = 0, nslot = 0;
  std::string err;
  const int r = scann::plan_tiles(b->mol_offset, b->n_struct, b->edge_offset, nullptr, b->n_atom, b->n_edge, tile_rows, tile_atoms, true,
                                  contiguous, part, big, row, &rows, &maxdeg, &nslot, err, false);
  if (r) {
    t_pack_error = "scann_plan_tiles_filled: " + err;
    return r;
  }
  const bool filled = scann::plan_tiles_filled(b->mol_offset, b->n_struct, b->edge_offset, b->n_atom, rows, tile_atoms, contiguous,
                                               (int32_t)big.size() / 3, atom_row, tile_offset, tiles);
  *n_tiles = (int32_t)tiles.size();
  if ((int32_t)tiles.size() > cap) return pack_fail("scann_plan_tiles_filled: output capacity too small");
  memcpy(atom_row_out, atom_row.data(), atom_row.size() * 4);
  memcpy(tile_offset_out, tile_offset.data(), tile_offset.size() * 4);
  memcpy(tiles_out, tiles.data(), tiles.size() * sizeof(scann::EdgeTile));
  return filled ? 1 : 0;
}

}
```

scann--material_amd/csrc/scann_runtime.cpp:

```cpp
#include "scann_runtime.h"

#include <mutex>

namespace {

struct BlockCache {
  std::multimap<size_t, void*> free_blocks;
  std::map<void*, size_t> size_of;
  size_t cached_bytes = 0;
};
std::map<int, BlockCache> g_block_cache;
std::mutex g_block_mu;
constexpr size_t BLOCK_CACHE_LIMIT = (size_t)16 << 30;
thread_local std::string g_create_error;

std::vector<WeightSpec> build_specs(const scann_config_t& c) {
  std::vector<WeightSpec> s;
  const int64_t d = c.local_dim, dg = c.global_dim, dout = c.dense_out, emb = c.embedding_dim;
  if (c.feature_cgcnn) {
    s.push_back({"embed_atom/kernel", 92, emb});
    s.push_back({"embed_atom/bias", emb, 0});
  } else {
    s.push_back({"embed_atom/embeddings", c.n_atoms, emb});
  }
// ... 299 lines not shown
  double least = 0.0;
  Row cen = first_centres(&least);
  if (least < SMALL_OPERAND) return "dense_embed: its swish output rows (the first layer's centres)" + few;
  if (c.g_update && L > 0) {
    Row g = filter_size("neighbor_d", (double)c.gaussian_d);
    const Row gw = filter_size("neighbor_w", 2.0 * M_PI);
    for (int k = 0; k < D; ++k) g[k] *= gw[k];
    if (small(g)) return "neighbor_d, neighbor_w: the products of their swish outputs (the first layer's geometry)" + few;
  }
  for (int i = 0; i < L; ++i) {
    const std::string p = "local_attention_" + std::to_string(i) + "/", r = "residual_norm_" + std::to_string(i) + "/";
    {
      Row ang = c.g_update ? ln_size(p + "layer_norm_g") : filter_size(p + "filter_geo", (double)c.gaussian_d);
      for (int k = 0; k < D; ++k) ang[k] *= cen[k];
      if (small(ang)) return p + "key: its operand rows (centres x geometry, component by component)" + few;
      cen = ln_size((c.use_attn_norm ? r : p) + "layer_norm");
    }
    std::vector<std::string> names = {p + "query/kernel", p + "key/kernel"};
    if (c.use_attn_norm) names.insert(names.end(), {r + "dense_1/kernel", r + "dense_2/kernel"});
    for (const std::string& n : names)
      if (col_small(n, 0)) return n + column;
    if (c.g_update) {
      for (int j = 0; j < 3; ++j)
        if (col_small(p + "filter_geo/kernel", j * D)) return p + "filter_geo/kernel, rows " + std::to_string(j * D) + ".." + std::to_string(j * D + D - 1) + column;
      if (ln_small(p + "layer_norm_g")) return p + "layer_norm_g: its output rows (the geometry) stay below 2^-8, where a split-fp16 operand keeps too few bits";
    }
    if (ln_small(p + "layer_norm")) return p + "layer_norm: its output rows (the context) stay below 2^-8, where a split-fp16 operand keeps too few bits";
    if (c.use_attn_norm) {
      if (ln_small(r + "layer_norm")) return r + "layer_norm: its output rows (the centres) stay below 2^-8, where a split-fp16 operand keeps too few bits";
      if (swish_small(p + "layer_norm", r + "dense_1"))
        return r + "dense_1: its swish output rows (the operand of dense_2) stay below 2^-8, where a split-fp16 operand keeps too few bits";
    }
  }
  for (const char* n : {"after_Lc/kernel", "global_attention/query/kernel", "global_attention/key/kernel"})
    if (col_small(n, 0)) return n + column;
  if (L > 0 && swish_small((c.use_attn_norm ? "residual_norm_" : "local_attention_") + std::to_string(L - 1) + "/layer_norm", "after_Lc"))
    return "after_Lc: its swish output rows (the operand of global_attention/query and key) stay below 2^-8, where a split-fp16 operand keeps too few bits";
  return "";
}

}

extern "C" {

int scann_abi_version(void) { return SCANN_ABI_VERSION; }

int scann_device_count(void) {
  int n = 0;
  if (hipGetDeviceCount(&n) != hipSuccess) return 0;
  return n;
}

const char* scann_last_error(const scann_handle_t* h) { return h ? h->err.c_str() : g_create_error.c_str(); }

int scann_create(const scann_config_t* cfg, int device_id, scann_handle_t** out) {
  if (!cfg || !out) return fail(nullptr, SCANN_ERR_INVALID, "scann_create: null argument");
  *out = nullptr;
  if (cfg->n_gauss != NG) return fail(nullptr, SCANN_ERR_UNSUPPORTED, "scann_create: 20 Gaussians (custom_layers.py:39-53 as called by scann_model.py:378,384)");
  const bool generic = cfg->local_dim != D || cfg->global_dim != D || cfg->dense_out != D || cfg->num_head != NHEAD ||
                       (getenv("SCANN_GENERIC") && atoi(getenv("SCANN_GENERIC")));
  if (generic) {
    if (cfg->local_dim <= 0 || cfg->num_head <= 0 || cfg->global_dim <= 0 || cfg->dense_out <= 0 || cfg->local_dim % cfg->num_head != 0)
      return fail(nullptr, SCANN_ERR_INVALID, "scann_create: local_dim must be a positive multiple of num_head (attention.py:170-173), global_dim and dense_out positive");
    if (cfg->local_dim > 1024 || cfg->global_dim > 1024 || cfg->dense_out > 1024 || cfg->embedding_dim > 1024)
      return fail(nullptr, SCANN_ERR_UNSUPPORTED, "scann_create: widths above 1024 are not implemented");
  } else if (cfg->embedding_dim + (cfg->use_ring ? 10 : 0) > 160) {
    return fail(nullptr, SCANN_ERR_UNSUPPORTED, "scann_create: embedding_dim (+10 ring features) must be <= 160");
  }
  if (cfg->n_atoms <= 0 || cfg->embedding_dim <= 0 || cfg->n_attention < 0 || !(cfg->gaussian_d > 0))
    return fail(nullptr, SCANN_ERR_INVALID, "scann_create: bad hyper-parameter");
  int ndev = 0;
  if (hipGetDeviceCount(&ndev) != hipSuccess || ndev <= 0)
    return fail(nullptr, SCANN_ERR_NO_DEVICE, "scann_create: no HIP device visible (this library has no CPU fallback)");
  if (device_id < 0 || device_id >= ndev) return fail(nullptr, SCANN_ERR_NO_DEVICE, "scann_create: device_id out of range");
  scann_handle* h = new scann_handle();
  h->cfg = *cfg;
  h->generic = generic;
  h->device = device_id;
  h->specs = build_specs(*cfg);
  if (const char* xr = getenv("SCANN_XCD_REMAP")) h->xcd_remap = atoi(xr) != 0;
  if (const char* ar = getenv("SCANN_ATOM_ROWS")) h->atom_rows = atoi(ar);
  if (const char* fb = getenv("SCANN_FUSE_BASIS")) h->fuse_basis = atoi(fb) != 0;
  if (const char* tf = getenv("SCANN_TILE_FILL")) h->tile_fill = atoi(tf) != 0;
  if (const char* st = getenv("SCANN_SPECIES_TABLES")) h->species_tables = atoi(st) != 0;
  if (const char* sg = getenv("SCANN_STRICT_RANGE")) h->strict_range = atoi(sg) != 0;
  if (const char* fe = getenv("SCANN_EXACT")) h->force_exact = atoi(fe) != 0;
  {
    hipDeviceProp_t prop;
    if (hipGetDeviceProperties(&prop, device_id) == hipSuccess && prop.multiProcessorCount > 0) h->n_cu = prop.multiProcessorCount;
  }
  if (const char* ns = getenv("SCANN_STREAMS")) h->nstream = std::min(MAX_STREAM, std::max(1, atoi(ns)));
  if (hipSetDevice(device_id) != hipSuccess) {
    delete h;
    return fail(nullptr, SCANN_ERR_HIP, "scann_create: hipSetDevice failed");
  }
  if (hipHostMalloc((void**)&h->range_flag, 128, hipHostMallocDefault) != hipSuccess) {
    delete h;
    return fail(nullptr, SCANN_ERR_HIP, "scann_create: hipHostMalloc failed");
  }
  for (int i = 0; i < 32; ++i) h->range_flag[i] = 0;
  for (int i = 0; i < h->nstream; ++i) {
    if (hipStreamCreateWithFlags(&h->streams[i], hipStreamNonBlocking) != hipSuccess) {
      delete h;
      return fail(nullptr, SCANN_ERR_HIP, "scann_create: hipStreamCreate failed");
    }
  }
  *out = h;
  return SCANN_OK;
}

void scann_destroy(scann_handle_t* h) {
  if (!h) return;
  (void)hipSetDevice(h->device);
  (void)hipDeviceSynchronize();
  for (int i = 0; i < MAX_STREAM; ++i)
    if (h->streams[i]) (void)hipStreamDestroy(h->streams[i]);
  if (h->d_weights) (void)hipFree(h->d_weights);
  for (scann_handle::DlStage& st : h->dl_stage)
    if (st.p) (void)hipHostFree(st.p);
  if (h->g_weights) (void)hipFree(h->g_weights);
  if (h->g_centres) (void)hipFree(h->g_centres);
  if (h->g_WT) (void)hipFree(h->g_WT);
  if (h->d_gt_descs) (void)hipFree(h->d_gt_descs);
  if (h->sp_c) (void)hipFree(h->sp_c);
  for (scann_handle::Stage& st : h->stage) {
    if (st.p) (void)hipHostFree(st.p);
    if (st.ev) (void)hipEventDestroy(st.ev);
  }
  if (h->copy_stream) (void)hipStreamDestroy(h->copy_stream);
  for (void* q : {(void*)h->t_master, (void*)h->t_grad, (void*)h->t_m, (void*)h->t_v, (void*)h->t_l2, (void*)h->t_descs, (void*)h->ig_grad})
    if (q) (void)hipFree(q);
  if (h->comm) ncclCommDestroy(h->comm);
  if (h->train_aux && !h->train_aux_borrowed) (void)hipStreamDestroy(h->train_aux);
  if (h->h_stat) (void)hipHostFree(h->h_stat);
  if (h->range_flag) (void)hipHostFree(h->range_flag);
  for (float* t : h->h_targets)
    if (t) (void)hipHostFree(t);
  for (hipEvent_t e : h->step_ev)
    if (e) (void)hipEventDestroy(e);
  if (h->train_aux2) (void)hipStreamDestroy(h->train_aux2);
  for (hipEvent_t e : h->train_ev) (void)hipEventDestroy(e);
  for (hipEvent_t e : h->time_ev) (void)hipEventDestroy(e);
  free_models(h->models);
  if (h->sc_db) free_batch(h->sc_db);
  if (h->sc_arena) (void)hipFree(h->sc_arena);
  if (h->pp_dev) (void)hipFree(h->pp_dev);
  if (h->pp_host) (void)hipHostFree(h->pp_host);
  if (h->sc_host) (void)hipHostFree(h->sc_host);
  cache_release(h->device);
  delete h;
}

int scann_num_streams(const scann_handle_t* h) { return h ? h->nstream : 0; }

int scann_weight_count(const scann_handle_t* h) { return h ? (int)h->specs.size() : SCANN_ERR_INVALID; }

int scann_weight_name(const scann_handle_t* h, int index, const char** name, int64_t* rows, int64_t* cols) {
  if (!h || index < 0 || index >= (int)h->specs.size()) return SCANN_ERR_INVALID;
  if (name) *name = h->specs[index].name.c_str();
  if (rows) *rows = h->specs[index].rows;
  if (cols) *cols = h->specs[index].cols;
  return SCANN_OK;
}

int64_t scann_param_count(const scann_handle_t* h) {
  if (!h) return SCANN_ERR_INVALID;
// ... 336 lines not shown
```

scann--material_amd/csrc/scann_runtime.h:

```cpp
#pragma once
#include "../../include/scann_hip.h"
#include "scann_internal.h"
#include "scann_train.h"

#include <rccl/rccl.h>

#include <algorithm>
#include <cmath>
#include <cstdlib>
#include <cstring>
#include <map>
#include <memory>
#include <string>
#include <vector>

using namespace scann;

namespace scann {

constexpr int MAX_STREAM = 16;

hipError_t cached_malloc(void** p, size_t bytes);
void cached_free(void* p);
void cache_release(int dev);
// ... 9 lines not shown
  float *Z = nullptr;
  float *T = nullptr;
  float *Gn = nullptr;
  float *K = nullptr, *q = nullptr;
  float *t1 = nullptr, *ctx = nullptr;
  float *pre1 = nullptr, *h1 = nullptr, *t2 = nullptr;
  float *cc_out = nullptr;
};
struct GenKeep {
  char* arena = nullptr;
  size_t bytes = 0;
  char* barena = nullptr;
  size_t bbytes = 0;
  std::vector<GenLayerKeep> layer;
  float *embE = nullptr, *ring10 = nullptr, *pre_e = nullptr, *cc0 = nullptr;
  float *gd = nullptr, *gw = nullptr, *pre_d = nullptr, *pre_w = nullptr, *Td = nullptr, *Tw = nullptr, *G0 = nullptr;
  float *cc_L = nullptr, *z_pre = nullptr, *z = nullptr, *gq = nullptr, *gk = nullptr, *rep = nullptr, *hid_pre = nullptr, *hid = nullptr;
  float drop_p = 0.f, attn_p = 0.f;
  unsigned long long seed = 0;
  std::map<std::string, std::pair<const float*, size_t>> dbg;
};

struct scann_train_ws {
  char* arena = nullptr;
  std::vector<float*> tA;
  float *keep_q = nullptr, *keep_V = nullptr, *keep_T = nullptr, *keep_ang = nullptr, *keep_K = nullptr;
  float *keep_pre1 = nullptr, *keep_H1 = nullptr, *keep_T2 = nullptr;
  float *keep_preA = nullptr, *keep_z = nullptr;
  std::vector<float*> tE;
  float *rep = nullptr, *dpre = nullptr, *dy = nullptr, *targets = nullptr, *dlut = nullptr;
  float* wpart = nullptr;
  size_t wpart_floats = 0;
  float* det_part = nullptr;
  size_t det_floats = 0;
  double* sse = nullptr;
  char* ig = nullptr;
  size_t ig_bytes = 0;
  float drop_p = 0.f, attn_p = 0.f;
  unsigned long long seed = 0;
  GenKeep gen;
  ~scann_train_ws() {
    cached_free(arena);
    cached_free(det_part);
    cached_free(ig);
    cached_free(gen.arena);
    cached_free(gen.barena);
  }
};

struct Timer;
struct ModelSet;
void free_models(ModelSet* ms);

struct McState {
  const McRow* rows;
  unsigned long long seed;
  uint32_t t;
  float p_drop, p_attn;
};

}

struct scann_handle {
  scann_config_t cfg{};
  int device = 0;
  std::string err;
  hipStream_t streams[MAX_STREAM]{};
  int nstream = 2;
  std::vector<WeightSpec> specs;
  bool loaded = false;
  bool debug = false;
  uint64_t out_layers = 0;
  int32_t out_flags = 0;
  int tile_atoms = TQ;
  int n_cu = 256;
  int time_every = 0;
  int64_t time_count = 0;
  std::vector<hipEvent_t> time_ev;
  std::vector<int> time_edges;
  int xcd_remap = 1;
  int atom_rows = 0;
  int fuse_basis = 1;
  int tile_fill = 1;
  int species_tables = 1;
  bool generic = false;
  float* g_weights = nullptr;
  float* g_centres = nullptr;
  std::map<std::string, int64_t> g_off;
  std::vector<GenTransDesc> gt_descs;
  GenTransDesc* d_gt_descs = nullptr;
  std::map<std::string, int64_t> gt_off;
  float* g_WT = nullptr;
  int gt_max = 0;
  bool weights_exact = false;
  bool small_operands = false;
  std::string exact_reason;
  bool force_exact = false;
  bool strict_range = false;
  int64_t exact_reruns = 0;
  float* d_weights = nullptr;
  std::vector<LayerParams> layers;
  HeadParams head{};
  BasisParams basis{};
  const float* lut = nullptr;
  float *sp_c = nullptr, *sp_P1 = nullptr, *sp_P3 = nullptr, *sp_q = nullptr;
  bool sp_dirty = true;
  const float* cd = nullptr;
  EmbedArgs embed{};
  std::vector<float> host_master;
  std::vector<int64_t> spec_off;
  std::vector<RepackDesc> descs;
  size_t arena_floats = 0, o_lut = 0, o_emb = 0, o_Wde = 0, o_bde = 0;
  struct LayerT {
    const float *W1T, *W2T, *W3T, *WqT, *WkT, *Wf1T, *Wf2T;
    const _Float16 *W1Th, *W2Th, *W3Th, *WqTh, *WkTh, *Wf1Th, *Wf2Th;
  };
  std::vector<LayerT> layersT;
  const float *WaT = nullptr, *WgqT = nullptr, *WgkT = nullptr;
  const _Float16* WaTh = nullptr;
  float *t_master = nullptr, *t_grad = nullptr, *t_m = nullptr, *t_v = nullptr, *t_l2 = nullptr;
  RepackDesc* t_descs = nullptr;
  float* ig_grad = nullptr;
  int64_t t_step = 0;
  float attn_drop_p = 0.f;
  bool deterministic = false;
  ncclComm_t comm = nullptr;
  double* h_stat = nullptr;
  float* h_targets[3] = {nullptr, nullptr, nullptr};
  size_t h_targets_cap[3] = {0, 0, 0};
  hipEvent_t step_ev[2] = {nullptr, nullptr};
  int64_t step_begun = 0, step_ended = 0;
  bool grads_zeroed = false;
  struct Stage { char* p = nullptr; size_t cap = 0; hipEvent_t ev = nullptr; bool used = false; };
  static constexpr int N_STAGE = 8;
  Stage stage[N_STAGE];
  int stage_next = 0;
  struct PadScratch { std::vector<int32_t> gidx, at, mol, eoff, col; std::vector<float> dist, wgt, ga; };
  PadScratch pad_scratch;
  struct DlStage { char* p = nullptr; size_t cap = 0; };
  DlStage dl_stage[MAX_STREAM];
  hipStream_t copy_stream = nullptr;
  hipStream_t train_aux2 = nullptr;
  bool train_fused = true;
  bool train_aux_borrowed = false;
  hipStream_t train_aux = nullptr;
  std::vector<hipEvent_t> train_ev;
  char* sc_arena = nullptr;
  size_t sc_cap = 0;
  char* pp_host = nullptr;
  char* pp_dev = nullptr;
  size_t pp_cap = 0;
  char* sc_host = nullptr;
  size_t sc_host_cap = 0;
  struct scann_dbatch* sc_db = nullptr;
  int comm_world = 1;
  int32_t* range_flag = nullptr;
  ModelSet* models = nullptr;
  uint64_t models_gen = 0;
};

struct scann_dbatch {
  int32_t n_struct = 0, n_atom = 0, n_edge = 0, n_tile = 0, max_atoms = 0, tile_rows = 64, max_degree = 0, tile_atoms = TQ;
  char* arena = nullptr;
  int32_t *atomic = nullptr, *mol_offset = nullptr, *edge_offset = nullptr, *edge_col = nullptr, *edge_row = nullptr;
  float *dist = nullptr, *weight = nullptr, *ring = nullptr, *cgcnn = nullptr, *c0 = nullptr;
  EdgeTile* tiles = nullptr;
// ... 130 lines not shown
```

scann--material_amd/scann/_hip.py:

```python
from __future__ import annotations

import ctypes as C
import os

import numpy as np

_HERE = os.path.dirname(os.path.abspath(__file__))
LIB_PATH = os.environ.get("SCANN_HIP_LIB") or os.path.join(os.path.dirname(_HERE), "lib", "libscann_hip.so")

SCANN_OK = 0
STATUS = {0: "OK", -1: "INVALID", -2: "UNSUPPORTED", -3: "NO_DEVICE", -4: "HIP", -5: "WEIGHTS", -6: "OOM", -7: "RANGE"}


class ScannHipError(RuntimeError):
    def __init__(self, code, msg):
        super().__init__("libscann_hip: %s (%d): %s" % (STATUS.get(code, "?"), code, msg))
        self.code, self.detail = code, msg


class Config(C.Structure):
    _fields_ = [
        ("n_atoms", C.c_int32), ("embedding_dim", C.c_int32), ("local_dim", C.c_int32), ("num_head", C.c_int32),
        ("n_attention", C.c_int32), ("global_dim", C.c_int32), ("dense_out", C.c_int32), ("n_gauss", C.c_int32),
        ("gaussian_d", C.c_float), ("g_update", C.c_int32), ("use_attn_norm", C.c_int32), ("use_ga_norm", C.c_int32),
        ("use_ring", C.c_int32), ("feature_cgcnn", C.c_int32), ("relu_out", C.c_int32),
    ]


class TensorDesc(C.Structure):
    _fields_ = [("name", C.c_char_p), ("offset", C.c_int64), ("numel", C.c_int64)]


class Batch(C.Structure):
    _fields_ = [
        ("n_struct", C.c_int32), ("n_atom", C.c_int32), ("n_edge", C.c_int32),
        ("atomic", C.c_void_p), ("mol_offset", C.c_void_p), ("edge_offset", C.c_void_p), ("edge_col", C.c_void_p),
        ("edge_dist", C.c_void_p), ("edge_weight", C.c_void_p), ("ring", C.c_void_p), ("cgcnn", C.c_void_p),
    ]


class Profile(C.Structure):
    _fields_ = [
        ("ms_basis", C.c_float), ("ms_atom", C.c_float), ("ms_edge", C.c_float), ("ms_readout", C.c_float),
        ("ms_total", C.c_float), ("n_edge_launch", C.c_int32), ("n_atom_launch", C.c_int32), ("reserved", C.c_int32),
    ]


_P = C.c_void_p
SYMBOLS = [
    ("scann_abi_version", C.c_int, []),
    ("scann_device_count", C.c_int, []),
    ("scann_create", C.c_int, [C.POINTER(Config), C.c_int, C.POINTER(_P)]),
    ("scann_destroy", None, [_P]),
    ("scann_last_error", C.c_char_p, [_P]),
    ("scann_weight_count", C.c_int, [_P]),
    ("scann_weight_name", C.c_int, [_P, C.c_int, C.POINTER(C.c_char_p), C.POINTER(C.c_int64), C.POINTER(C.c_int64)]),
    ("scann_load_weights", C.c_int, [_P, _P, C.POINTER(TensorDesc), C.c_int]),
    ("scann_forward", C.c_int, [_P, C.POINTER(Batch), _P, _P]),
    ("scann_forward_padded", C.c_int, [_P, C.c_int32, C.c_int32, C.c_int32, _P, _P, _P, _P, _P, _P, _P, _P]),
    ("scann_batch_upload", C.c_int, [_P, C.POINTER(Batch), C.POINTER(_P)]),
    ("scann_batch_free", None, [_P, _P]),
    ("scann_batch_release", None, [_P, _P]),
    ("scann_forward_resident", C.c_int, [_P, _P, C.c_int]),
    ("scann_batch_download", C.c_int, [_P, _P, _P, _P]),
    ("scann_sync", C.c_int, [_P]),
    ("scann_num_streams", C.c_int, [_P]),
    ("scann_forward_profile", C.c_int, [_P, _P, C.POINTER(Profile)]),
    ("scann_edge_timing", C.c_int, [_P, C.c_int]),
    ("scann_edge_timing_read", C.c_int, [_P, C.POINTER(C.c_double), C.POINTER(C.c_int64), C.POINTER(C.c_double)]),
    ("scann_set_debug", C.c_int, [_P, C.c_int]),
    ("scann_debug_read", C.c_int, [_P, _P, C.c_int, C.c_int, _P]),
    ("scann_train_debug_read", C.c_int64, [_P, _P, C.c_char_p, _P, C.c_int64]),
    ("scann_debug_stamps", C.c_int, [_P, _P, _P, C.c_int]),
    ("scann_param_count", C.c_int64, [_P]),
    ("scann_train_begin", C.c_int, [_P]),
    ("scann_train_forward", C.c_int, [_P, _P, _P, C.c_float, C.c_uint64, C.POINTER(C.c_double)]),
    ("scann_train_backward", C.c_int, [_P, _P, C.c_double, C.c_int64]),
    ("scann_set_attention_dropout", C.c_int, [_P, C.c_float]),
    ("scann_set_deterministic", C.c_int, [_P, C.c_int]),
    ("scann_zero_grads", C.c_int, [_P]),
    ("scann_allreduce_grads", C.c_int, [_P]),
    ("scann_allreduce_sse", C.c_int, [_P, C.POINTER(C.c_double), C.POINTER(C.c_int64)]),
    ("scann_adam_step", C.c_int, [_P, C.c_float, C.c_float, C.c_float, C.c_float, C.c_float]),
    ("scann_train_step", C.c_int, [_P, _P, _P, C.c_float, C.c_uint64] + [C.c_float] * 5 + [C.POINTER(C.c_double), C.POINTER(C.c_int64)]),
    ("scann_train_step_begin", C.c_int, [_P, _P, _P, C.c_float, C.c_uint64] + [C.c_float] * 5),
    ("scann_train_step_end", C.c_int, [_P, C.POINTER(C.c_double), C.POINTER(C.c_int64), C.POINTER(C.c_double)]),
    ("scann_get_grads", C.c_int, [_P, _P]),
    ("scann_get_weights", C.c_int, [_P, _P]),
    ("scann_comm_unique_id", C.c_int, [C.c_char_p]),
    ("scann_comm_init", C.c_int, [_P, C.c_char_p, C.c_int, C.c_int]),
    ("scann_comm_ranks", C.c_int, [_P]),
    ("scann_broadcast_weights", C.c_int, [_P, C.c_int]),
    ("scann_pack_last_error", C.c_char_p, []),
    ("scann_pack_padded", C.c_int, [C.c_int32, C.c_int32, C.c_int32] + [_P] * 17 + [C.POINTER(C.c_int32), C.POINTER(C.c_int32)]),
    ("scann_slice_count", C.c_int, [_P, _P, _P, C.c_int32, C.c_int64, C.POINTER(C.c_int64), C.POINTER(C.c_int64)]),
    ("scann_slice_batch", C.c_int, [_P] * 8 + [C.c_int32, C.c_int64] + [_P] * 7),
    ("scann_plan_tiles", C.c_int, [C.POINTER(Batch), C.c_int32, C.c_int32, C.c_int32, C.c_int32, _P, _P, C.POINTER(C.c_int32), C.POINTER(C.c_int32)]),
    ("scann_plan_tiles_filled", C.c_int, [C.POINTER(Batch), C.c_int32, C.c_int32, C.c_int32, _P, _P, _P, C.POINTER(C.c_int32)]),
    ("scann_batch_tile_plan", C.c_int, [_P, _P, _P]),
    ("scann_exact_reruns", C.c_int64, [_P]),
    ("scann_weights_exact", C.c_int, [_P]),
    ("scann_device_memory", C.c_int, [_P, C.POINTER(C.c_int64), C.POINTER(C.c_int64)]),
    ("scann_batch_info", C.c_int, [_P, _P, _P]),
    ("scann_count_padded", C.c_int, [C.c_int32, C.c_int32, C.c_int32, _P, C.c_int32, _P, C.c_int32, _P, _P, _P, C.POINTER(C.c_int32), C.POINTER(C.c_int32)]),
    ("scann_upload_padded", C.c_int, [_P, C.c_int32, C.c_int32, C.c_int32, _P, _P, C.c_int32, _P, _P, C.c_int32, _P, _P, C.POINTER(_P),
                                      C.POINTER(C.c_int32), C.POINTER(C.c_int32)]),
    ("scann_batch_read_csr", C.c_int, [_P, _P, _P, _P, _P, _P, _P, _P]),
    ("scann_host_copy", C.c_int, [_P, _P, C.c_int64]),
    ("scann_set_outputs", C.c_int, [_P, C.c_uint64, C.c_int32]),
    ("scann_output_read", C.c_int64, [_P, _P, C.c_int32, C.c_int32, _P, C.c_int64]),
    ("scann_input_grads", C.c_int, [_P, _P, _P, _P, _P, _P, _P]),
    ("scann_predict_mc", C.c_int, [_P, _P, C.c_int32, C.c_uint64, _P, C.c_float, C.c_float, _P, _P, _P, _P, _P]),
    ("scann_mc_drop_scale", C.c_double, [C.c_uint64, C.c_int32, C.c_uint64, C.c_uint32, C.c_uint64, C.c_float]),
    ("scann_ablate_pooling", C.c_int, [_P, _P, C.c_int32, _P, _P, _P, _P]),
    ("scann_shapley", C.c_int, [_P, _P, C.c_int32, C.c_uint64, _P, _P, _P, _P, _P, _P, _P, _P, _P, _P]),
    ("scann_shapley_profile", C.c_int, [_P, _P, C.c_int32, C.c_uint64, _P, _P]),
    ("scann_shapley_permutation", None, [C.c_uint64, C.c_uint64, C.c_int32, C.c_int32, _P]),
    ("scann_shapley_reduce_host", C.c_int, [_P, _P, _P, C.c_int32, C.c_int32, _P, _P, _P, _P]),
    ("scann_rollout_floats", C.c_int64, [_P, _P]),
    ("scann_attention_rollout", C.c_int, [_P, _P, C.c_float, C.c_int32, C.c_int32, _P, _P, _P, _P]),
    ("scann_index_create", C.c_int, [_P, C.c_int32, C.POINTER(_P)]),
    ("scann_index_free", None, [_P, _P]),
    ("scann_index_size", C.c_int64, [_P]),
    ("scann_index_add", C.c_int, [_P, _P, _P, C.c_int64, _P, _P]),
    ("scann_index_read", C.c_int, [_P, _P, C.c_int64, C.c_int64, _P, _P, _P]),
    ("scann_index_query", C.c_int, [_P, _P, _P, C.c_int64, _P, C.c_int32, _P, _P, _P, _P]),
    ("scann_index_add_batch", C.c_int, [_P, _P, _P, C.c_int32, _P]),
    ("scann_index_query_batch", C.c_int, [_P, _P, _P, C.c_int32, _P, C.c_int32, _P, _P, _P, _P, _P, _P]),
    ("scann_knn_distsq", C.c_float, [_P, _P, C.c_int64]),
    ("scann_knn_distsq_matrix", None, [_P, C.c_int64, _P, C.c_int64, C.c_int64, _P]),
    ("scann_index_segments", C.c_int64, [_P, _P, _P, _P]),
    ("scann_index_match", C.c_int, [_P, _P, _P, _P, C.c_int64, _P, C.c_int32, C.c_int32, _P, _P, _P, _P, _P, _P, _P]),
    ("scann_index_match_batch", C.c_int, [_P, _P, _P, _P, C.c_int32, C.c_int32, _P, _P, _P, _P, _P, _P, _P, _P, _P]),
    ("scann_match_parts_host", C.c_int, [_P, _P, C.c_int64, _P, _P, C.c_int64, C.c_int64, _P]),
    ("scann_index_pairing", C.c_int, [_P, _P, _P, _P, C.c_int64, _P, _P, C.c_int64, _P, _P, _P, _P, _P]),
    ("scann_index_pairing_batch", C.c_int, [_P, _P, _P, _P, C.c_int32, C.c_int32, C.c_int32] + [_P] * 12),
    ("scann_pairing_host", C.c_int, [_P, C.c_int64, _P, C.c_int64, C.c_int64, _P, _P, _P, _P, _P]),
    ("scann_pairing_solve_host", C.c_int, [_P, C.c_int32, _P, _P]),
    ("scann_index_select", C.c_int64, [_P, _P, _P, C.c_int64, C.c_float, _P, _P, _P, _P]),
    ("scann_kcenter_host", C.c_int64, [_P, C.c_int64, _P, C.c_int64, C.c_int64, C.c_int64, C.c_float, _P, _P]),
    ("scann_index_kmeans", C.c_int64, [_P, _P, C.c_int32, _P, _P, C.c_int32, C.c_int64, _P, _P, _P, _P, _P]),
    ("scann_kmeans_host", C.c_int64, [_P, C.c_int64, C.c_int64, C.c_int32, _P, C.c_int32, C.c_int64, _P, _P, _P, _P, _P]),
    ("scann_index_moments", C.c_int, [_P, _P, _P, _P, _P, _P, _P]),
    ("scann_index_project", C.c_int, [_P, _P, C.c_int64, C.c_int64, _P, _P, _P, C.c_int32, _P, _P, _P]),
    ("scann_project_batch", C.c_int, [_P, _P, C.c_int32, _P, _P, _P, C.c_int32, _P, _P, _P, _P, _P]),
    ("scann_moments_host", C.c_int, [_P, C.c_int64, C.c_int64, _P, _P, _P, _P, _P]),
    ("scann_project_host", C.c_int, [_P, C.c_int64, C.c_int64, _P, _P, _P, C.c_int32, _P, _P, _P]),
    ("scann_sym_eig_host", C.c_int, [_P, C.c_int64, _P, _P, _P]),
    ("scann_pca_bits", C.c_int, [C.c_int64]),
    ("scann_index_fit_moments", C.c_int, [_P, _P, _P, C.c_int32, _P, _P, _P, _P, _P]),
    ("scann_index_ridge_loo", C.c_int, [_P, _P, _P, C.c_int32, _P, _P, _P, C.c_int32, _P, _P, C.c_int32, C.c_float, _P, _P, _P, _P, _P, _P, _P]),
    ("scann_ridge_loo_host", C.c_int, [_P, C.c_int64, C.c_int64, _P, C.c_int32, _P, _P, _P, C.c_int32, _P, _P, C.c_int32, C.c_float, _P, _P, _P, _P, _P,
                                       _P, _P]),
    ("scann_head_batch", C.c_int, [_P, _P, C.c_int32, _P, _P, _P, C.c_int32, _P, C.c_int32, _P, C.c_float, _P, _P, _P, _P]),
    ("scann_rbf_weight", C.c_float, [C.c_float, C.c_float]),
    ("scann_rbf_weight_array", None, [_P, C.c_int64, C.c_float, _P]),
    ("scann_index_rbf_features", C.c_int, [_P, _P, _P, C.c_int32, C.c_float, _P]),
    ("scann_rbf_features_host", C.c_int, [_P, C.c_int64, C.c_int64, _P, C.c_int32, C.c_float, _P]),
    ("scann_rbf_head_batch", C.c_int, [_P, _P, C.c_int32, _P, C.c_int32, C.c_float, _P, _P, _P, C.c_int32, _P, C.c_int32, _P, C.c_float, _P, _P, _P,
                                       _P, _P]),
    ("scann_index_logit_pass", C.c_int, [_P, _P, _P, C.c_int32, _P, _P, C.c_int32, _P, C.c_int32, _P, _P, _P, _P, _P]),
    ("scann_logit_pass_host", C.c_int, [_P, C.c_int64, C.c_int64, _P, C.c_int32, _P, _P, C.c_int32, _P, C.c_int32, _P, _P, _P, _P, _P]),
    ("scann_logit_head_batch", C.c_int, [_P, _P, C.c_int32, _P, _P, C.c_int32, _P, _P, _P]),
    ("scann_embed_iterate", C.c_int, [_P, C.c_int64, _P, _P, _P, _P, _P, _P, C.c_int32, C.c_float, C.c_float, C.c_float, C.POINTER(C.c_double), _P]),
    ("scann_embed_iterate_host", C.c_int, [C.c_int64, _P, _P, _P, _P, _P, _P, C.c_int32, C.c_float, C.c_float, C.c_float, C.POINTER(C.c_double), _P]),
    ("scann_index_density", C.c_int, [_P, _P, _P, C.c_int64, _P, C.c_float, _P]),
    ("scann_index_peaks", C.c_int, [_P, _P, C.c_float, _P, _P, _P]),
    ("scann_index_density_batch", C.c_int, [_P, _P, _P, C.c_int32, C.c_float, _P, _P, _P]),
    ("scann_density_host", C.c_int, [_P, C.c_int64, C.c_int64, _P, C.c_int64, _P, C.c_float, _P]),
    ("scann_peaks_host", C.c_int, [_P, C.c_int64, C.c_int64, C.c_float, _P, _P, _P]),
    ("scann_index_mst", C.c_int, [_P, _P, _P, _P, _P, _P, _P, _P]),
    ("scann_mst_host", C.c_int, [_P, C.c_int64, C.c_int64, _P, _P, _P, _P, _P]),
    ("scann_mst_last_rounds", C.c_int, [C.c_int32, _P, _P, _P, _P]),
    ("scann_index_silhouette", C.c_int, [_P, _P, _P, C.c_int32, _P, C.c_int64, C.c_int32, C.c_int32, _P, _P, _P, _P, _P]),
    ("scann_silhouette_host", C.c_int, [_P, C.c_int64, C.c_int64, _P, C.c_int32, _P, C.c_int64, C.c_int32, C.c_int32, C.c_int32, _P, _P, _P, _P, _P]),
    ("scann_index_ranks", C.c_int, [_P, _P, _P, C.c_int64, _P, C.c_int32, _P, _P]),
    ("scann_ranks_host", C.c_int, [_P, C.c_int64, C.c_int64, _P, C.c_int64, _P, C.c_int32, C.c_int32, _P, _P]),
    ("scann_index_partition", C.c_int, [_P, _P, C.c_int32, C.c_int32, _P]),
    ("scann_index_partition_args", C.c_int, [_P, _P, _P]),
    ("scann_index_cells_read", C.c_int, [_P, _P, _P, _P, _P, _P, _P, _P]),
    ("scann_index_search_stats", C.c_int, [_P, _P]),
    ("scann_index_query_rows", C.c_int, [_P, _P, C.c_int64, C.c_int64, C.c_int32, _P, _P, _P, _P]),
    ("scann_cells_capacity", C.c_int64, [C.c_int64, C.c_int32]),
    ("scann_cells_host", C.c_int, [_P, C.c_int64, C.c_int64, C.c_int32, C.c_int32, _P, _P, _P, _P, _P, _P]),
    ("scann_index_within", C.c_int, [_P, _P, _P, C.c_int64, _P, C.c_float, C.c_int64, _P, _P, _P, _P, _P, _P]),
    ("scann_index_within_rows", C.c_int, [_P, _P, C.c_int64, C.c_int64, C.c_int32, C.c_float, C.c_int64, _P, _P, _P, _P, _P, _P]),
    ("scann_index_within_batch", C.c_int, [_P, _P, _P, C.c_int32, _P, C.c_float, C.c_int64, _P, _P, _P, _P, _P, _P, _P, _P]),
    ("scann_within_host", C.c_int, [_P, C.c_int64, C.c_int64, _P, _P, C.c_int64, _P, _P, C.c_int32, C.c_float, C.c_int64, _P, _P, _P, _P]),
    ("scann_cell_bound", C.c_double, [C.c_float, C.c_float, C.c_float]),
# ... 910 lines not shown


def mst_last_rounds():
    comp, sec, skip, tiles = np.zeros(40, np.int32), np.zeros(40, np.float64), np.zeros(40, np.int64), np.zeros(1, np.int64)
    n = int(load_library().scann_mst_last_rounds(40, _ptr(comp), _ptr(sec), _ptr(skip), _ptr(tiles)))
    return {"components": comp[:n].copy(), "seconds": sec[:n].copy(), "skipped": skip[:n].copy(), "tiles": int(tiles[0])}


def check_rollout_args(residual, head, depth, num_head, n_attention):
    try:
        residual = float(residual)
    except (TypeError, ValueError):
        raise ValueError("residual must be a number in [0, 1], got %r" % (residual,)) from None
    if not 0.0 <= residual <= 1.0:
        raise ValueError("residual must lie in [0, 1], got %r" % (residual,))
    for name, v, lo, hi in (("head", head, 0, int(num_head) - 1), ("depth", depth, 1, int(n_attention))):
        if v is None:
            continue
        if isinstance(v, bool) or not isinstance(v, (int, np.integer)) or not lo <= int(v) <= hi:
            raise ValueError("%s must be None or an integer in %d .. %d, got %r" % (name, lo, hi, v))
    return residual, -1 if head is None else int(head), 0 if depth is None else int(depth)


_lib = None
_pinned = False


def _hw_queue_advice(n, fix):
    if n <= 4:
        return None
    return ("GPU_MAX_HW_QUEUES=%d: with more than 4 hardware queues a stream waiting on a later-created stream stalls ~2 ms "
            "per wait (trainer.fit: 3x slower, profiles/r03_notes.md); %s" % (n, "SCANN_FIX_HW_QUEUES=1: unset, ROCm's default applies to "
            "this process (effective only if HIP has not started yet)" if fix else "left as set -- SCANN_FIX_HW_QUEUES=1 unsets it"))


def _check_hw_queues():
    v = os.environ.get("GPU_MAX_HW_QUEUES")
    if not v:
        return
    try:
        n = int(v)
    except ValueError:
        return
    fix = os.environ.get("SCANN_FIX_HW_QUEUES") == "1"
    msg = _hw_queue_advice(n, fix)
    if msg:
        import warnings

        warnings.warn(msg, RuntimeWarning, stacklevel=3)
        if fix:
            del os.environ["GPU_MAX_HW_QUEUES"]


def _check_runtime_env():
    bad = []
    if os.environ.get("HIP_FORCE_DEV_KERNARG") == "0":
        bad.append("HIP_FORCE_DEV_KERNARG=0")
    if os.environ.get("AMD_OPT_FLUSH") not in (None, "", "1"):
        bad.append("AMD_OPT_FLUSH=%s" % os.environ["AMD_OPT_FLUSH"])
    if os.environ.get("GPU_FLUSH_ON_EXECUTION") not in (None, "", "0"):
        bad.append("GPU_FLUSH_ON_EXECUTION=%s" % os.environ["GPU_FLUSH_ON_EXECUTION"])
    if bad:
        import warnings

        warnings.warn("%s in the environment: measured 4-40 %% slower forwards and up to 2x slower training steps on MI355X than the "
                      "HIP runtime's defaults (profiles/r04_notes.md)" % ", ".join(bad), RuntimeWarning, stacklevel=3)


def load_library(path=None):
    global _lib
    if _lib is not None and path is None:
        return _lib
    p = path or LIB_PATH
    if not os.path.exists(p):
        raise OSError(
            "libscann_hip.so not found at %s -- build it with `python -c 'import __graft_entry__ as g; g.build()'` "
            "or `make -C scann--material_amd/csrc`; this package has no CPU fallback" % p)
    if int(os.environ.get("WORLD_SIZE", "1") or 1) > 1:
        os.environ.setdefault("HSA_ENABLE_IPC_MODE_LEGACY", "0")
    _check_hw_queues()
    _check_runtime_env()
    lib = C.CDLL(p)
    for name, res, args in SYMBOLS:
        if name in ("scann_plan_tiles_filled", "scann_batch_tile_plan", "scann_weights_exact") and os.environ.get("SCANN_HIP_LIB") and not hasattr(lib, name):
            continue
        fn = getattr(lib, name)
        fn.restype = res
        fn.argtypes = args
    if lib.scann_abi_version() != 1:
        raise OSError("libscann_hip.so ABI version mismatch")
    if path is None:
        _lib = lib
    return lib


def comm_unique_id():
    buf = C.create_string_buffer(128)
    rc = load_library().scann_comm_unique_id(buf)
    if rc != SCANN_OK:
        raise ScannHipError(rc, "scann_comm_unique_id failed")
    return buf.raw


def mc_drop_scale(seed, t, key, tag, idx, p):
    return float(load_library().scann_mc_drop_scale(int(seed) & 0xFFFFFFFFFFFFFFFF, int(t), int(key) & 0xFFFFFFFFFFFFFFFF, int(tag), int(idx),
                                                    float(p)))


def _ptr(a):
    return a.ctypes.data if a is not None else None


def shapley_permutation(seed, key, p, n):
    out = np.empty(max(int(n), 0), np.int32)
    load_library().scann_shapley_permutation(int(seed) & 0xFFFFFFFFFFFFFFFF, int(key) & 0xFFFFFFFFFFFFFFFF, int(p), int(n), _ptr(out))
    return out


def shapley_reduce_host(values, perms, mol_offset, baseline):
    values = np.ascontiguousarray(values, dtype=np.float32)
    perms = np.ascontiguousarray(perms, dtype=np.int32)
    mol = np.ascontiguousarray(mol_offset, dtype=np.int32)
    base = np.ascontiguousarray(baseline, dtype=np.float64)
    B, A = mol.shape[0] - 1, int(mol[-1])
    if values.ndim != 2 or values.shape != perms.shape or values.shape[1] != A or base.shape != (B,):
        raise ValueError("values / perms must be [P, %d] and baseline [%d]" % (A, B))
    sh, se, full = np.empty(A, np.float64), np.empty(A, np.float64), np.empty(B, np.float64)
    lib = load_library()
    r = lib.scann_shapley_reduce_host(_ptr(values), _ptr(perms), _ptr(mol), B, values.shape[0], _ptr(base), _ptr(sh), _ptr(se), _ptr(full))
    if r != 0:
        raise ScannHipError(r, (lib.scann_last_error(None) or b"").decode())
    return sh, se, full


class PackedBatch:

    def __init__(self, atomic, mol_offset, edge_offset, edge_col, edge_dist, edge_weight, pad_shape=None, gidx=None,
                 ring=None, cgcnn=None):
        self.atomic = np.ascontiguousarray(atomic, dtype=np.int32) if atomic is not None else None
        self.ring = np.ascontiguousarray(ring, dtype=np.float32) if ring is not None else None
        self.cgcnn = np.ascontiguousarray(cgcnn, dtype=np.float32) if cgcnn is not None else None
        self.mol_offset = np.ascontiguousarray(mol_offset, dtype=np.int32)
        self.edge_offset = np.ascontiguousarray(edge_offset, dtype=np.int32)
        self.edge_col = np.ascontiguousarray(edge_col, dtype=np.int32)
        self.edge_dist = np.ascontiguousarray(edge_dist, dtype=np.float32)
        self.edge_weight = np.ascontiguousarray(edge_weight, dtype=np.float32)
        self.pad_shape = pad_shape
        self.atom_mask = gidx

    @property
    def n_struct(self):
        return int(self.mol_offset.shape[0] - 1)

    @property
    def n_atom(self):
        return int(self.edge_offset.shape[0] - 1)

    @property
    def n_edge(self):
        return int(self.edge_col.shape[0])

    def as_struct(self):
        return Batch(self.n_struct, self.n_atom, self.n_edge, _ptr(self.atomic), _ptr(self.mol_offset),
                     _ptr(self.edge_offset), _ptr(self.edge_col), _ptr(self.edge_dist), _ptr(self.edge_weight),
                     _ptr(self.ring), _ptr(self.cgcnn))

    def repad_ga(self, ga_packed):
        return ga_packed if self.pad_shape is None else repad_atoms(ga_packed, self.atom_mask)[..., None]


def concat_packed(parts):
    parts = list(parts)
    a_off = np.cumsum([0] + [p.n_atom for p in parts])
    e_off = np.cumsum([0] + [p.n_edge for p in parts])
    cat = lambda xs: np.concatenate(xs) if all(x is not None for x in xs) else None
    return PackedBatch(
        cat([p.atomic for p in parts]),
        np.concatenate([[0]] + [p.mol_offset[1:].astype(np.int64) + a_off[i] for i, p in enumerate(parts)]),
        np.concatenate([[0]] + [p.edge_offset[1:].astype(np.int64) + e_off[i] for i, p in enumerate(parts)]),
        np.concatenate([p.edge_col.astype(np.int64) + a_off[i] for i, p in enumerate(parts)]),
        np.concatenate([p.edge_dist for p in parts]), np.concatenate([p.edge_weight for p in parts]),
        ring=cat([p.ring for p in parts]), cgcnn=cat([p.cgcnn for p in parts]))


def slice_packed(pk, s0, s1):
    a0, a1 = int(pk.mol_offset[s0]), int(pk.mol_offset[s1])
    e0, e1 = int(pk.edge_offset[a0]), int(pk.edge_offset[a1])
    part = lambda x: x[a0:a1] if x is not None else None
    return PackedBatch(part(pk.atomic), pk.mol_offset[s0:s1 + 1] - a0, pk.edge_offset[a0:a1 + 1] - e0, pk.edge_col[e0:e1] - a0,
                       pk.edge_dist[e0:e1], pk.edge_weight[e0:e1], ring=part(pk.ring), cgcnn=part(pk.cgcnn))


def pack_inputs(inputs):
    lib = load_library()
    atomic = np.asarray(inputs["atomic"])
    cgcnn = None
    if atomic.ndim == 3:
        cgcnn, atomic = np.ascontiguousarray(atomic, dtype=np.float32), None
        if cgcnn.shape[2] != 92:
            raise ValueError("cgcnn features must be [B, M, 92]")
    else:
        atomic = np.ascontiguousarray(atomic, dtype=np.int32)
    amask = np.asarray(inputs["atom_mask"])
    if amask.ndim == 3:
        amask = amask[..., 0]
    amask = np.ascontiguousarray(amask != 0)
    nbr = np.ascontiguousarray(inputs["neighbors"], dtype=np.int32)
    nmask = np.ascontiguousarray(np.asarray(inputs["neighbor_mask"]) != 0)
    B, M = amask.shape
    if nbr.ndim != 3 or nbr.shape[:2] != (B, M) or nmask.shape != nbr.shape or \
            (atomic is not None and atomic.shape != (B, M)) or (cgcnn is not None and cgcnn.shape[:2] != (B, M)):
        raise ValueError("inconsistent input shapes")
    N = nbr.shape[2]
    dist = np.ascontiguousarray(inputs["neighbor_distance"], dtype=np.float32)
    wgt = np.ascontiguousarray(inputs["neighbor_weight"], dtype=np.float32)
    ring = np.ascontiguousarray(inputs["ring_aromatic"], dtype=np.float32) if "ring_aromatic" in inputs else None
    if dist.shape != nbr.shape or wgt.shape != nbr.shape or (ring is not None and ring.shape != (B, M, 2)):
        raise ValueError("inconsistent input shapes")
    o_atomic = np.empty(B * M, np.int32) if atomic is not None else None
    o_cgcnn = np.empty((B * M, 92), np.float32) if cgcnn is not None else None
    o_ring = np.empty((B * M, 2), np.float32) if ring is not None else None
    o_mol, o_eoff = np.empty(B + 1, np.int32), np.empty(B * M + 1, np.int32)
    o_col, o_dist, o_wgt = np.empty(B * M * N, np.int32), np.empty(B * M * N, np.float32), np.empty(B * M * N, np.float32)
    row_of = np.empty(B * M, np.int32)
    na, ne = C.c_int32(0), C.c_int32(0)
    rc = lib.scann_pack_padded(B, M, N, _ptr(atomic), _ptr(cgcnn), _ptr(amask), _ptr(nbr), _ptr(nmask), _ptr(wgt), _ptr(dist),
                               _ptr(ring), _ptr(o_atomic), _ptr(o_cgcnn), _ptr(o_ring), _ptr(o_mol), _ptr(o_eoff), _ptr(o_col),
                               _ptr(o_dist), _ptr(o_wgt), _ptr(row_of), C.byref(na), C.byref(ne))
    if rc != SCANN_OK:
        raise ValueError((lib.scann_pack_last_error() or b"").decode())
    na, ne = na.value, ne.value
    return PackedBatch(o_atomic[:na] if o_atomic is not None else None, o_mol, o_eoff[:na + 1], o_col[:ne], o_dist[:ne],
                       o_wgt[:ne], pad_shape=(B, M), gidx=amask, ring=o_ring[:na] if o_ring is not None else None,
                       cgcnn=o_cgcnn[:na] if o_cgcnn is not None else None)


def plan_tiles(packed, tile_rows=64, tile_atoms=24, allow_chunks=True):
    lib = load_library()
    cap = packed.n_atom + packed.n_edge // 32 + 2
    tiles, part = np.empty((cap, 4), np.int32), np.empty(cap, np.int32)
    nt, ns = C.c_int32(0), C.c_int32(0)
    st = packed.as_struct()
    rc = lib.scann_plan_tiles(C.byref(st), tile_rows, tile_atoms, int(allow_chunks), cap, _ptr(tiles), _ptr(part), C.byref(nt), C.byref(ns))
    if rc < 0:
        raise ScannHipError(rc, (lib.scann_pack_last_error() or b"").decode())
    return rc, tiles[:nt.value].copy(), part[:nt.value].copy(), ns.value


def plan_tiles_filled(packed, tile_rows=64, tile_atoms=24):
    lib = load_library()
    cap = packed.n_atom + packed.n_edge // 32 + 2
    atom_row, tile_offset = np.empty(packed.n_atom, np.int32), np.empty(packed.n_atom + 1, np.int32)
    tiles = np.empty((cap, 4), np.int32)
    nt = C.c_int32(0)
    st = packed.as_struct()
    rc = lib.scann_plan_tiles_filled(C.byref(st), tile_rows, tile_atoms, cap, _ptr(atom_row), _ptr(tile_offset), _ptr(tiles), C.byref(nt))
    if rc < 0:
        raise ScannHipError(rc, (lib.scann_pack_last_error() or b"").decode())
    return bool(rc), atom_row, tile_offset, tiles[:nt.value].copy()


def slice_dataset(ds_mol_offset, ds_edge_offset, ds_atomic, ds_ring, ds_edge_local, ds_edge_dist, ds_edge_weight, sel):
    lib = load_library()
    sel = np.ascontiguousarray(sel, dtype=np.int64)
    n_total = int(ds_mol_offset.shape[0] - 1)
    na, ne = C.c_int64(0), C.c_int64(0)
    if lib.scann_slice_count(_ptr(ds_mol_offset), _ptr(ds_edge_offset), _ptr(sel), len(sel), n_total, C.byref(na), C.byref(ne)) != SCANN_OK:
        raise ValueError((lib.scann_pack_last_error() or b"").decode())
    na, ne = na.value, ne.value
    o_atomic, o_mol, o_eoff = np.empty(na, np.int32), np.empty(len(sel) + 1, np.int32), np.empty(na + 1, np.int32)
    o_ring = np.empty((na, 2), np.float32) if ds_ring is not None else None
    o_col, o_dist, o_wgt = np.empty(ne, np.int32), np.empty(ne, np.float32), np.empty(ne, np.float32)
    rc = lib.scann_slice_batch(_ptr(ds_mol_offset), _ptr(ds_edge_offset), _ptr(ds_atomic), _ptr(ds_ring), _ptr(ds_edge_local),
                               _ptr(ds_edge_dist), _ptr(ds_edge_weight), _ptr(sel), len(sel), n_total, _ptr(o_atomic),
                               _ptr(o_ring), _ptr(o_mol), _ptr(o_eoff), _ptr(o_col), _ptr(o_dist), _ptr(o_wgt))
    if rc != SCANN_OK:
        raise ValueError((lib.scann_pack_last_error() or b"").decode())
    return PackedBatch(o_atomic, o_mol, o_eoff, o_col, o_dist, o_wgt, ring=o_ring)


def repad_local_attention(attn, atom_mask, neighbor_mask):
    amask = np.asarray(atom_mask).reshape(np.shape(neighbor_mask)[:2]) != 0
    em = (np.asarray(neighbor_mask) != 0) & amask[:, :, None]
    B, M, N = em.shape
    attn = np.asarray(attn, dtype=np.float32)
    H = attn.shape[1]
    if attn.shape[0] != int(em.sum()):
        raise ValueError("%d attention rows for %d real neighbour slots" % (attn.shape[0], int(em.sum())))
    out = np.zeros((B, M, N, H), dtype=np.float32)
    if N:
        out[~em.any(-1)] = np.float32(1.0) / np.float32(N)
    out[em] = attn
    return np.ascontiguousarray(out.transpose(0, 3, 1, 2))


def repad_edges(x, atom_mask, neighbor_mask):
    em = np.asarray(neighbor_mask) != 0
    em = em & (np.asarray(atom_mask).reshape(em.shape[:2]) != 0)[:, :, None]
    x = np.asarray(x, dtype=np.float32)
    if x.shape[0] != int(em.sum()):
        raise ValueError("%d edge values for %d real neighbour slots" % (x.shape[0], int(em.sum())))
    out = np.zeros(em.shape, dtype=np.float32)
    out[em] = x
    return out


def repad_atoms(x, atom_mask, fill=0, dtype=None):
    amask = np.asarray(atom_mask)
    amask = amask.reshape(amask.shape[:2]) != 0
    x = np.asarray(x)
    out = np.full(amask.shape + x.shape[1:], fill, dtype=dtype or (x.dtype if x.dtype.kind in "iu" else np.float32))
    out[amask] = x
    return out


def _mask_arg(m):
    m = np.asarray(m)
    if m.dtype in (np.bool_, np.uint8, np.int8):
        return np.ascontiguousarray(m), 1
    if m.dtype == np.float32:
        return np.ascontiguousarray(m), 4
    return np.ascontiguousarray(m != 0), 1


def _mask_bytes(m):
    m, size = _mask_arg(m)
    return (m if size == 1 else np.ascontiguousarray(m != 0)).view(np.uint8)


def count_padded(inputs):
    lib = load_library()
    amask, asz = _mask_arg(inputs["atom_mask"])
    nmask, nsz = _mask_arg(inputs["neighbor_mask"])
    B, M, N = nmask.shape
    mol, eoff, row_of = np.empty(B + 1, np.int32), np.empty(B * M + 1, np.int32), np.empty(B * M, np.int32)
    na, ne = C.c_int32(0), C.c_int32(0)
    if lib.scann_count_padded(B, M, N, _ptr(amask), asz, _ptr(nmask), nsz, _ptr(mol), _ptr(eoff), _ptr(row_of), C.byref(na), C.byref(ne)) != SCANN_OK:
        raise ValueError((lib.scann_pack_last_error() or b"").decode())
    return mol, eoff[:na.value + 1], row_of.reshape(B, M)
# ... 88 lines not shown
            pass

    def weight_specs(self):
        out = []
        for i in range(self.lib.scann_weight_count(self._h)):
            name, r, c = C.c_char_p(), C.c_int64(), C.c_int64()
            self._check(self.lib.scann_weight_name(self._h, i, C.byref(name), C.byref(r), C.byref(c)))
            out.append((name.value.decode(), (r.value, c.value) if c.value else (r.value,)))
        return out

    def _weight_blob(self, weights):
        specs = self.weight_specs()
        chunks, descs, off = [], [], 0
        names = []
        for name, shape in specs:
            if name not in weights:
                raise ScannHipError(-5, "missing tensor " + name)
            t = np.ascontiguousarray(weights[name], dtype=np.float32)
            if tuple(t.shape) != tuple(shape):
                raise ScannHipError(-5, "tensor %s has shape %s, expected %s" % (name, t.shape, shape))
            chunks.append(t.ravel())
            names.append(name.encode())
            descs.append((names[-1], off, t.size))
            off += t.size
        blob = np.concatenate(chunks).astype(np.float32)
        arr = (TensorDesc * len(descs))(*[TensorDesc(n, o, s) for n, o, s in descs])
        return blob, arr, len(descs), names

    def models_load(self, members, relu_out=None):
        K = len(members)
        if not 1 <= K <= 16:
            raise ValueError("a model set holds 1 to 16 members, not %d" % K)
        parts = [self._weight_blob(w) for w in members]
        blobs = (_P * K)(*[b.ctypes.data for b, _, _, _ in parts])
        mans = (_P * K)(*[C.cast(a, _P) for _, a, _, _ in parts])
        ns = np.array([n for _, _, n, _ in parts], dtype=np.int32)
        relu = None if relu_out is None else np.ascontiguousarray(np.asarray(relu_out, dtype=np.int32).reshape(-1))
        if relu is not None and relu.shape[0] != K:
            raise ValueError("relu_out: %d flags for %d members" % (relu.shape[0], K))
        self._check(self.lib.scann_models_load(self._h, K, blobs, mans, _ptr(ns), _ptr(relu)))
        self.n_models = K

    def models_count(self):
        return int(self.lib.scann_models_count(self._h))

    def forward_models(self, rb, slot=0):
        self._check(self.lib.scann_forward_models(self._h, rb._h, int(slot)))

    def models_download(self, rb, want_ga=True):
        K = self.models_count()
        y = np.empty((K, rb.packed.n_struct), dtype=np.float32)
        ga = np.empty((K, rb.packed.n_atom), dtype=np.float32) if want_ga else None
        self._check(self.lib.scann_models_download(self._h, rb._h, _ptr(y), _ptr(ga)))
        return y, ga

    def load_weights(self, weights):
        blob, arr, n, _names = self._weight_blob(weights)
        self._check(self.lib.scann_load_weights(self._h, _ptr(blob), arr, n))

    def forward(self, packed, want_ga=True):
        y = np.empty(packed.n_struct, dtype=np.float32)
        ga = np.empty(packed.n_atom, dtype=np.float32) if want_ga else None
        st = packed.as_struct()
        self._check(self.lib.scann_forward(self._h, C.byref(st), _ptr(y), _ptr(ga)))
        return y, ga

    def forward_padded(self, inputs, want_ga=True):
        atomic = np.ascontiguousarray(inputs["atomic"], dtype=np.int32)
        B, M = atomic.shape
        amask = _mask_bytes(np.asarray(inputs["atom_mask"]).reshape(B, M))
        nbr = np.ascontiguousarray(inputs["neighbors"], dtype=np.int32)
        N = nbr.shape[2]
        nmask = _mask_bytes(inputs["neighbor_mask"])
        wgt = np.ascontiguousarray(inputs["neighbor_weight"], dtype=np.float32)
        dst = np.ascontiguousarray(inputs["neighbor_distance"], dtype=np.float32)
        if nbr.shape != (B, M, N) or nmask.shape != nbr.shape or wgt.shape != nbr.shape or dst.shape != nbr.shape:
            raise ValueError("inconsistent input shapes")
        y = np.empty(B, dtype=np.float32)
        ga = np.empty((B, M, 1), dtype=np.float32) if want_ga else None
        self._check(self.lib.scann_forward_padded(self._h, B, M, N, _ptr(atomic), _ptr(amask), _ptr(nbr), _ptr(nmask),
                                                  _ptr(wgt), _ptr(dst), _ptr(y), _ptr(ga)))
        return y, ga

    def upload(self, packed):
        st = packed.as_struct()
        db = _P()
        self._check(self.lib.scann_batch_upload(self._h, C.byref(st), C.byref(db)))
        return ResidentBatch(self, packed, db)

    def upload_padded(self, inputs):
        atomic = np.ascontiguousarray(inputs["atomic"], dtype=np.int32)
        B, M = atomic.shape
        amask, asz = _mask_arg(np.asarray(inputs["atom_mask"]).reshape(B, M))
        nbr = np.ascontiguousarray(inputs["neighbors"], dtype=np.int32)
        N = nbr.shape[2]
        nmask, nsz = _mask_arg(inputs["neighbor_mask"])
        wgt = np.ascontiguousarray(inputs["neighbor_weight"], dtype=np.float32)
        dst = np.ascontiguousarray(inputs["neighbor_distance"], dtype=np.float32)
        if nbr.shape != (B, M, N) or nmask.shape != nbr.shape or wgt.shape != nbr.shape or dst.shape != nbr.shape or amask.shape != (B, M):
            raise ValueError("inconsistent input shapes")
        db, na, ne = _P(), C.c_int32(0), C.c_int32(0)
        self._check(self.lib.scann_upload_padded(self._h, B, M, N, _ptr(atomic), _ptr(amask), asz, _ptr(nbr), _ptr(nmask), nsz, _ptr(wgt),
                                                 _ptr(dst), C.byref(db), C.byref(na), C.byref(ne)))
        return ResidentBatch(self, PaddedInfo(B, na.value, ne.value, amask != 0 if amask.dtype != np.bool_ else amask), db)

    def read_csr(self, rb):
        p = rb.packed
        atomic, mol, eoff = np.empty(p.n_atom, np.int32), np.empty(p.n_struct + 1, np.int32), np.empty(p.n_atom + 1, np.int32)
        col, dist, wgt = np.empty(p.n_edge, np.int32), np.empty(p.n_edge, np.float32), np.empty(p.n_edge, np.float32)
        self._check(self.lib.scann_batch_read_csr(self._h, rb._h, _ptr(atomic), _ptr(mol), _ptr(eoff), _ptr(col), _ptr(dist), _ptr(wgt)))
        return {"atomic": atomic, "mol_offset": mol, "edge_offset": eoff, "edge_col": col, "edge_dist": dist, "edge_weight": wgt}

    def forward_resident(self, rb, slot=0):
        self._check(self.lib.scann_forward_resident(self._h, rb._h, int(slot)))

    def download(self, rb, want_ga=True):
        y = np.empty(rb.packed.n_struct, dtype=np.float32)
        ga = np.empty(rb.packed.n_atom, dtype=np.float32) if want_ga else None
        self._check(self.lib.scann_batch_download(self._h, rb._h, _ptr(y), _ptr(ga)))
        return y, ga

    def sync(self):
        self._check(self.lib.scann_sync(self._h))

    def set_outputs(self, attn_layers=(), after_lc=False, bf_property=False):
        bits = 0
        for k in attn_layers:
            k = int(k)
            if not 0 <= k < 64:
                raise ValueError("local_attention layer %d out of range" % k)
            bits |= 1 << k
        flags = (OUT_AFTER_LC if after_lc else 0) | (OUT_BF_PROPERTY if bf_property else 0)
        self._check(self.lib.scann_set_outputs(self._h, bits, flags))

    def read_output(self, rb, what, layer=0):
        p = rb.packed
        rows, cols = {OUT_LOCAL_ATTENTION: (p.n_edge, self.cfg.num_head), OUT_AFTER_LC: (p.n_atom, self.cfg.global_dim),
                      OUT_BF_PROPERTY: (p.n_struct, self.cfg.dense_out)}[what]
        out = np.empty((rows, cols), dtype=np.float32)
        n = self.lib.scann_output_read(self._h, rb._h, int(what), int(layer), _ptr(out), out.size)
        if n < 0:
            self._check(int(n))
        assert n == out.size, (n, out.shape)
        return out

    def exact_reruns(self):
        return int(self.lib.scann_exact_reruns(self._h))

    def weights_exact(self):
        if not hasattr(self.lib, "scann_weights_exact"):
            return False
        return bool(self.lib.scann_weights_exact(self._h))

    def device_memory(self):
        f, t = C.c_int64(0), C.c_int64(0)
        self._check(self.lib.scann_device_memory(self._h, C.byref(f), C.byref(t)))
        return int(f.value), int(t.value)

    def batch_info(self, rb):
        out = np.zeros(8, dtype=np.int32)
        self._check(self.lib.scann_batch_info(self._h, rb._h, _ptr(out)))
        keys = ("structs", "atoms", "edges", "big_atoms", "merge_slots", "max_degree", "tiles", "tile_rows")
        return dict(zip(keys, (int(v) for v in out)))

    def tile_plan(self, rb):
        out = np.zeros(2, dtype=np.int32)
        self._check(self.lib.scann_batch_tile_plan(self._h, rb._h, _ptr(out)))
        return bool(out[0]), int(out[1])

    def num_streams(self):
        return self.lib.scann_num_streams(self._h)

    def profile(self, rb):
        p = Profile()
        self._check(self.lib.scann_forward_profile(self._h, rb._h, C.byref(p)))
        return {k: getattr(p, k) for k, _ in Profile._fields_ if k != "reserved"}

    def input_grads(self, rb, distance=True, weight=True, ring=False, cgcnn=False):
        p = rb.packed
        y = np.empty(p.n_struct, dtype=np.float32)
        out = {"neighbor_distance": np.empty(p.n_edge, np.float32) if distance else None,
               "neighbor_weight": np.empty(p.n_edge, np.float32) if weight else None,
               "ring_aromatic": np.empty((p.n_atom, 2), np.float32) if ring else None,
               "atomic": np.empty((p.n_atom, 92), np.float32) if cgcnn else None}
        self._check(self.lib.scann_input_grads(self._h, rb._h, _ptr(y), _ptr(out["neighbor_distance"]), _ptr(out["neighbor_weight"]),
                                               _ptr(out["ring_aromatic"]), _ptr(out["atomic"])))
# ... 611 lines not shown
```

scann--material_amd/scann/models/scann_model.py:

```python
from __future__ import annotations

import contextlib
import functools
import io
import json
import os

import numpy as np

from .. import _hip
from .latent_index import (EMBED_NEIGHBOURS, LatentClassHead, LatentClustering, LatentEmbedding, LatentHead, LatentHierarchy, LatentIndex, LatentKernelHead,
                           LatentProjection, batch_jobs, check_min_cluster_size, count_structures, density_of_sums, embed_fit_args, hierarchy_fit_args, level_dim, peaks_fit_args,
                           stop_dist2_of)

INPUT_NAMES = ["atomic", "atom_mask", "neighbors", "neighbor_mask", "neighbor_weight", "neighbor_distance"]

_MODEL_DEFAULTS = dict(feature="atomic", use_ring=False, use_drop=False, g_update=False, gaussian_d=4.0,
                       use_attn_norm=True, use_ga_norm=True)
_HYPER_DEFAULTS = dict(scaler=False, scheduler="cosine", use_ref=False, target="", pretrained="", deterministic=False)


def normalize_config(config):
    config.setdefault("model", {})
    config.setdefault("hyper", {})
# ... 709 lines not shown
               "predict_property_std": np.concatenate([p["y_std"] for p in parts]).reshape(-1, 1)}
        amask = inputs.atom_mask if packed_in else inputs["atom_mask"]
        for name, key in (("global_attention", "ga_mean"), ("global_attention_std", "ga_std")):
            ga = np.concatenate([p[key] for p in parts])
            out[name] = ga.reshape(-1, 1) if amask is None else _hip.repad_atoms(ga, amask)[..., None]
        if return_samples:
            out["samples"] = np.concatenate([p["y_samples"] for p in parts], axis=1)[:, :, None]
        return out

    BIG_PREDICT = 1024
    PREDICT_CHUNK = 2048
    BIG_SLOTS = 6_000_000

    def _select(self, sel):
        if sel is None:
            self.engine.set_outputs()
        else:
            self.engine.set_outputs(sel[1], after_lc=sel[2], bf_property=sel[3])

    def _pipeline(self, jobs, finish, sel=None, launch=None):
        eng = self.engine
        ns = eng.num_streams()
        launch = launch or eng.forward_resident
        pending = []
        rb = None

        def fetch_oldest():
            finish(*pending[0])
            pending.pop(0)[0].release()

        try:
            if sel is not None:
                self._select(sel)
            for k, (upload, tag) in enumerate(jobs):
                rb = upload()
                if len(pending) >= 2 * ns:
                    fetch_oldest()
                launch(rb, k % ns)
                pending.append((rb, tag))
                rb = None
            while pending:
                fetch_oldest()
        finally:
            if rb is not None:
                rb.free()
            for b, _ in pending:
                b.free()
            if sel is not None:
                self._select(None)

    def _batch_size(self, batch_size):
        bs = int(self.config["hyper"]["batch_size"] if batch_size is None else batch_size)
        if bs < 1:
            raise ValueError("batch_size must be >= 1")
        return bs

    def _run_chunks(self, data, batch_size, call, host_pack=False):
        eng, parts, at = self.engine, [], [0]

        def finish(rb, cnt):
            parts.append(call(rb, at[0], at[0] + cnt))
            at[0] += cnt

        upload = (lambda chunk: eng.upload(_hip.pack_inputs(chunk))) if host_pack else None
        self._pipeline(batch_jobs(self, data, self._batch_size(batch_size), upload), finish, launch=lambda rb, slot: None)
        return parts

    def _run_cat(self, inputs, batch_size, call, empty):
        parts = self._run_chunks(inputs, batch_size, call)
        return {n: np.concatenate([p[n] for p in parts]) if parts else empty[n] for n in empty}

    @contextlib.contextmanager
    def _indexed(self, data, level, ids=None, batch_size=None):
        if isinstance(data, LatentIndex):
            data.check_model(self)
            yield data
            return
        index = self.build_index(data, level=level, ids=ids, batch_size=batch_size)
        try:
            yield index
        finally:
            index.free()

    def _upload_padded(self, inputs):
        m, eng = self.config["model"], self.engine
        if m["feature"] == "atomic" and not m["use_ring"] and not eng.training:
            return eng.upload_padded(inputs)
        return eng.upload(_hip.pack_inputs(inputs))

    def _read_outputs(self, rb, sel):
        eng, out = self.engine, {}
        for k in sel[1]:
            out["local_attention_%d" % k] = eng.read_output(rb, _hip.OUT_LOCAL_ATTENTION, k)
        if sel[2]:
            out["after_Lc"] = eng.read_output(rb, _hip.OUT_AFTER_LC)
        if sel[3]:
            out["bf_property"] = eng.read_output(rb, _hip.OUT_BF_PROPERTY)
        return out

    def _assemble(self, sel, y, ga_pad, packed, atom_mask=None, neighbor_mask=None):
        res = []
        for n in sel[0]:
            if n == "predict_property":
                res.append(y.reshape(-1, 1))
            elif n == "global_attention":
                res.append(ga_pad)
            elif n.startswith("local_attention_"):
                a = packed["local_attention_%d" % int(n[16:])]
                res.append(a if atom_mask is None else _hip.repad_local_attention(a, atom_mask, neighbor_mask))
            elif n == "after_Lc":
                res.append(packed[n] if atom_mask is None else _hip.repad_atoms(packed[n], atom_mask))
            else:
                res.append(packed[n])
        return res

    def _predict_outputs(self, inputs, sel):
        eng, got = self.engine, []
        is_packed = isinstance(inputs, _hip.PackedBatch)

        def finish(rb, _):
            y, ga = eng.download(rb, want_ga=True)
            got.extend((y, rb.packed.repad_ga(ga), self._read_outputs(rb, sel)))

        upload = functools.partial(eng.upload if is_packed else self._upload_padded, inputs)
        self._pipeline([(upload, None)], finish, sel)
        if is_packed:
            return self._assemble(sel, *got)
        return self._assemble(sel, *got, inputs["atom_mask"], inputs["neighbor_mask"])

    def _predict_chunked(self, inputs, sel=None):
        eng = self.engine
        B = len(inputs["atom_mask"])
        nb = np.shape(inputs["neighbors"])
        want_ga = self.infer if sel is None else "global_attention" in sel[0]
        outs = []
        C = min(self.PREDICT_CHUNK, max(512, -(-B // 4 // 128) * 128))
        C = max(1, min(C, (self.BIG_SLOTS * 2 // 3) // max(1, int(nb[1]) * max(1, int(nb[2])))))
        ys, gas = [], []

        def finish(rb, first):
            try:
                y, ga = eng.download(rb, want_ga=want_ga)
                if sel is not None:
                    outs.append(self._read_outputs(rb, sel))
            except _hip.ScannHipError as e:
                raise _hip.ScannHipError(e.code, "%s [structures %d..%d of this call]" % (e.detail, first, min(first + C, B) - 1)) from e
            ys.append(y)
            if want_ga:
                gas.append(ga)

        self._pipeline(((functools.partial(self._upload_padded, {key: v[i:i + C] for key, v in inputs.items()}), i)
                        for i in range(0, B, C)), finish, sel)
        y = np.concatenate(ys).reshape(-1, 1)
        if not want_ga and sel is None:
            return y
        amask = np.asarray(inputs["atom_mask"]).reshape(B, -1) != 0
        ga_pad = None
        if want_ga:
            ga_pad = _hip.repad_atoms(np.concatenate(gas), amask)[..., None]
        if sel is None:
            return [y, ga_pad]
        packed = {n: np.concatenate([o[n] for o in outs]) for n in (outs[0] if outs else {})}
        return self._assemble(sel, y, ga_pad, packed, amask, inputs["neighbor_mask"])

    @staticmethod
    def default_group(dataset):
        bs = int(getattr(dataset, "batch_size", 0) or 0)
        return max(1, 1024 // bs) if bs > 0 else 8

    def predict_dataset(self, dataset, group=None, want_ga=False, outputs=None):
        eng = self.engine
        ys, gas, ts = [], [], []
        group = int(group) if group else self.default_group(dataset)
        sel = None
        if outputs is not None:
            sel = _output_selection(outputs, int(self.config["model"]["n_attention"]))
            if "predict_property" in sel[0] or "global_attention" in sel[0]:
                raise ValueError("predict_dataset returns predict_property and global_attention as y and ga (want_ga=True)")
        per_struct = {n: [] for n in sel[0]} if sel is not None else None
        n = len(dataset)
        grouped = getattr(dataset, "batches", None)

        def jobs():
            for g0 in range(0, n, group):
                if grouped is not None:
                    pk, tgt = grouped(g0, min(n, g0 + group))
                    tg, counts = [np.asarray(tgt, dtype=np.float32)], None
                    if sel is not None:
                        bs = int(dataset.batch_size)
                        counts = [min(bs, pk.n_struct - j) for j in range(0, pk.n_struct, bs)]
                else:
                    parts, tg = [], []
                    for i in range(g0, min(n, g0 + group)):
                        item, tgt = dataset[i]
                        parts.append(item if isinstance(item, _hip.PackedBatch) else _hip.pack_inputs(item))
                        tg.append(np.asarray(tgt, dtype=np.float32))
                    pk = _hip.concat_packed(parts) if len(parts) > 1 else parts[0]
                    counts = [p.n_struct for p in parts]
                yield functools.partial(eng.upload, pk), (tg, pk, counts)

        def finish(rb, tag):
            tg, pk, counts = tag
            y, ga = eng.download(rb, want_ga=want_ga)
            if sel is not None:
                self._split_outputs(self._read_outputs(rb, sel), pk, counts, per_struct)
            ys.append(y)
            if want_ga:
                gas.append(ga)
            ts.extend(tg)

        self._pipeline(jobs(), finish, sel)
        if not ys:
            res = np.zeros(0, np.float32), (np.zeros(0, np.float32) if want_ga else None), np.zeros(0, np.float32)
        else:
            res = np.concatenate(ys), (np.concatenate(gas) if want_ga else None), np.concatenate(ts)
        return res if sel is None else res + (per_struct,)

    def _split_outputs(self, packed, pk, counts, per_struct):
        mol = np.asarray(pk.mol_offset, dtype=np.int64)
        eoff = np.asarray(pk.edge_offset, dtype=np.int64)
        deg = np.diff(eoff)
        s0 = 0
        for cnt in counts:
            a0, a1 = int(mol[s0]), int(mol[s0 + cnt])
            sizes = np.diff(mol[s0:s0 + cnt + 1])
            M = int(sizes.max()) if cnt else 0
            N = int(deg[a0:a1].max()) if a1 > a0 else 0
            st = np.repeat(np.arange(cnt), sizes)
            slot = np.arange(a1 - a0) - np.repeat(mol[s0:s0 + cnt] - a0, sizes)
            amask = np.zeros((cnt, M), dtype=bool)
            amask[st, slot] = True
            em = np.zeros((cnt, M, N), dtype=bool)
            em[st, slot] = np.arange(N)[None, :] < deg[a0:a1, None]
            for name, arr in packed.items():
                if name.startswith("local_attention_"):
                    v = _hip.repad_local_attention(arr[eoff[a0]:eoff[a1]], amask, em)
                elif name == "after_Lc":
                    v = _hip.repad_atoms(arr[a0:a1], amask)
                else:
                    v = arr[s0:s0 + cnt]
                per_struct[name].extend(list(v))
            s0 += cnt

    def summary(self):
        print("SCANN HIP model: %d parameters, %d local-attention layers, g_update=%s" % (
            self.count_params(), self.config["model"]["n_attention"], self.config["model"]["g_update"]))


def _read_container(path, config=None):
    with open(path, "rb") as f:
        magic = f.read(8)
    if magic.startswith(b"\x89HDF"):
        from .keras_import import load_keras_h5

        return load_keras_h5(path, config)
    z = np.load(path, allow_pickle=False)
    cfg = json.loads(str(z["__config__"]))
    return cfg, {k: z[k] for k in z.files if k != "__config__"}


def load_model(path, custom_objects=None, infer=False, config=None, outputs=None):
    cfg, weights = _read_container(path, config)
    if config is not None:
        cfg["hyper"].update({k: v for k, v in config.get("hyper", {}).items() if k != "target" or "target" not in cfg["hyper"]})
    return HipModel(cfg, weights, infer=infer, outputs=outputs)


def create_model_pretrained(pretrained):
    model = load_model(pretrained)
    model.summary()
    return model


def create_model(config, seed=None):
    model = HipModel(config, seed=seed)
    model.summary()
    return model


class SCANN:

    def __init__(self, config=None, pretrained="", mode="train"):
# ... 205 lines not shown
```

Baseline: 1.960 million.

## Plan filled edge tiles on host at upload with chunked multithreaded planner

```diff
diff --git a/include/scann_hip.h b/include/scann_hip.h
--- a/include/scann_hip.h
+++ b/include/scann_hip.h
@@ -95,6 +95,11 @@
                         int32_t atom_mask_size, const int32_t* neighbors, const void* neighbor_mask, int32_t neighbor_mask_size,
                         const float* neighbor_weight, const float* neighbor_distance, scann_dbatch_t** out, int32_t* n_atom_out,
                         int32_t* n_edge_out);
+int scann_batch_upload_once(scann_handle_t* h, const scann_batch_t* batch, scann_dbatch_t** out);
+int scann_upload_padded_once(scann_handle_t* h, int32_t B, int32_t M, int32_t N, const int32_t* atomic, const void* atom_mask,
+                             int32_t atom_mask_size, const int32_t* neighbors, const void* neighbor_mask, int32_t neighbor_mask_size,
+                             const float* neighbor_weight, const float* neighbor_distance, scann_dbatch_t** out, int32_t* n_atom_out,
+                             int32_t* n_edge_out);
 int scann_batch_read_csr(scann_handle_t* h, scann_dbatch_t* db, int32_t* atomic, int32_t* mol_offset, int32_t* edge_offset,
                          int32_t* edge_col, float* edge_dist, float* edge_weight);
 void scann_batch_free(scann_handle_t* h, scann_dbatch_t* db);
@@ -371,6 +376,8 @@
                      int32_t* tiles_out, int32_t* part_out, int32_t* n_tiles, int32_t* n_slots);
 int scann_plan_tiles_filled(const scann_batch_t* batch, int32_t tile_rows, int32_t tile_atoms, int32_t cap, int32_t* atom_row_out,
                             int32_t* tile_offset_out, int32_t* tiles_out, int32_t* n_tiles);
+int scann_plan_tiles_chunked(const scann_batch_t* batch, int32_t tile_rows, int32_t tile_atoms, int32_t chunk, int32_t n_threads,
+                             int32_t cap, int32_t* atom_row_out, int32_t* tile_offset_out, int32_t* tiles_out, int32_t* n_tiles);
 int scann_batch_tile_plan(scann_handle_t* h, const scann_dbatch_t* batch, int32_t* out2);
 
 #ifdef __cplusplus
diff --git a/scann--material_amd/csrc/scann_batch.cpp b/scann--material_amd/csrc/scann_batch.cpp
--- a/scann--material_amd/csrc/scann_batch.cpp
+++ b/scann--material_amd/csrc/scann_batch.cpp
@@ -18,7 +18,13 @@
 
 static inline void par_memcpy(void* dst, const void* src, size_t bytes) { (void)scann_host_copy(dst, src, (int64_t)bytes); }
 
-static int upload_impl(scann_handle_t* h, const scann_batch_t* b, scann_dbatch_t** out, bool scratch, const PaddedSrc* pad = nullptr) {
+constexpr double PLAN_NS_PER_TILE = 21.6, PLAN_NS_PER_ATOM = 5.5, PLAN_PAYS_AT = 0.5;
+static bool plan_pays(size_t n_tile, int rows, int32_t A, int32_t E, int L) {
+  return rows == TE_MAX && ((double)n_tile - (double)E / rows) * L * PLAN_NS_PER_TILE >= PLAN_PAYS_AT * A * PLAN_NS_PER_ATOM;
+}
+
+static int upload_impl(scann_handle_t* h, const scann_batch_t* b, scann_dbatch_t** out, bool scratch, const PaddedSrc* pad = nullptr,
+                       bool plan_fill = false) {
   if (!h || !b || !out) return fail(h, SCANN_ERR_INVALID, "scann_batch_upload: null argument");
   *out = nullptr;
   const int32_t B = b->n_struct, A = b->n_atom, E = b->n_edge;
@@ -67,7 +73,14 @@
   }
   const int32_t n_big = (int32_t)big_tab.size() / 3;
   const bool tile_side = h->cfg.g_update && !h->generic && E > 0;
-  const size_t n_ftile = tiles.size();
+  std::vector<int32_t> atom_row, tile_offset;
+  std::vector<EdgeTile> ftiles;
+  const bool planned = plan_fill && tile_side && h->tile_fill && n_big == 0 && tiles.size() > 1 &&
+                       (h->plan_at_upload < 0 ? plan_pays(tiles.size(), tile_rows, A, E, h->cfg.n_attention) : h->plan_at_upload != 0);
+  const bool filled = planned &&
+                      plan_tiles_filled(b->mol_offset, B, b->edge_offset, A, tile_rows, h->tile_atoms, tiles, n_big, atom_row, tile_offset,
+                                        ftiles, PLAN_CHUNK);
+  const size_t n_ftile = filled ? ftiles.size() : tiles.size();
   HIPCHK(h, hipSetDevice(h->device));
   scann_dbatch* db = nullptr;
   if (scratch) {
@@ -103,6 +116,8 @@
   const size_t o_col = take((size_t)E * 4), o_row = take((size_t)E * 4), o_dist = take((size_t)E * 4), o_wgt = take((size_t)E * 4);
   const size_t o_tiles = take(tiles.size() * sizeof(EdgeTile));
   const size_t o_tpart = take(n_big ? tiles.size() * 4 : 0), o_big = take((size_t)n_big * 3 * 4);
+  const size_t o_arow = take(filled ? (size_t)A * 4 : 0), o_toff = take(filled ? (size_t)(A + 1) * 4 : 0);
+  const size_t o_ftiles = take(filled ? n_ftile * sizeof(EdgeTile) : 0);
   const size_t o_inoff = take((size_t)(A + 1) * 4), o_inedge = take((size_t)E * 4);
   const size_t o_ring = take(h->cfg.use_ring ? (size_t)A * 2 * 4 : 0), o_cg = take(h->cfg.feature_cgcnn ? (size_t)A * 92 * 4 : 0);
   const size_t BM = pad ? (size_t)B * pad->M : 0, BMN = pad ? BM * pad->N : 0;
@@ -120,6 +135,8 @@
   const size_t o_pbuf = take((size_t)n_slot * 3 * D * 4);
   const size_t slot_bytes = tile_side ? n_ftile * TQ * 4 : 0;
   const size_t o_tatom = take(slot_bytes), o_te0 = take(slot_bytes), o_tsp = take(h->cfg.feature_cgcnn ? 0 : slot_bytes);
+  const size_t t_bytes = filled ? (size_t)E * 4 : 0;
+  const size_t o_tcol = take(t_bytes), o_trow = take(t_bytes), o_tdist = take(t_bytes), o_twgt = take(t_bytes);
   hipError_t e = hipSuccess;
   scann_handle::Stage* stage = nullptr;
   char* img_ptr = nullptr;
@@ -182,6 +199,11 @@
     memcpy(img.data() + o_wgt, b->edge_weight, (size_t)E * 4);
   }
   memcpy(img.data() + o_tiles, tiles.data(), tiles.size() * sizeof(EdgeTile));
+  if (filled) {
+    memcpy(img.data() + o_arow, atom_row.data(), (size_t)A * 4);
+    memcpy(img.data() + o_toff, tile_offset.data(), (size_t)(A + 1) * 4);
+    memcpy(img.data() + o_ftiles, ftiles.data(), n_ftile * sizeof(EdgeTile));
+  }
   const bool want_rev = h->t_master != nullptr;
   if (want_rev) {
     int32_t* in_off = reinterpret_cast<int32_t*>(img.data() + o_inoff);
@@ -216,6 +238,13 @@
     ta.tiles = (const EdgeTile*)(a0 + o_tiles); ta.n_tile = (int32_t)n_ftile; ta.n_atom = A;
     ta.edge_offset = d_eoff; ta.atomic = h->cfg.feature_cgcnn ? nullptr : (const int32_t*)(a0 + o_atomic);
     ta.tile_atom = (int32_t*)(a0 + o_tatom); ta.tile_edge0 = (int32_t*)(a0 + o_te0); ta.tile_species = (int32_t*)(a0 + o_tsp);
+    if (filled) {
+      ta.tiles = (const EdgeTile*)(a0 + o_ftiles);
+      ta.atom_row = (const int32_t*)(a0 + o_arow); ta.tile_offset = (const int32_t*)(a0 + o_toff);
+      ta.col = (const int32_t*)(a0 + o_col); ta.dist = (const float*)(a0 + o_dist); ta.weight = (const float*)(a0 + o_wgt);
+      ta.out_col = (int32_t*)(a0 + o_tcol); ta.out_row = (int32_t*)(a0 + o_trow);
+      ta.out_dist = (float*)(a0 + o_tdist); ta.out_weight = (float*)(a0 + o_twgt);
+    }
   }
   if (scratch) {
     if (e == hipSuccess) e = hipMemcpyAsync(db->arena, img.data(), in_bytes, hipMemcpyHostToDevice, h->streams[0]);
@@ -253,6 +282,12 @@
   if (tile_side) {
     db->tile_atom = (int32_t*)(a0 + o_tatom); db->tile_edge0 = (int32_t*)(a0 + o_te0);
     db->tile_species = h->cfg.feature_cgcnn ? nullptr : (int32_t*)(a0 + o_tsp);
+  }
+  db->fill_tried = planned;
+  if (filled) {
+    db->filled = true;
+    db->f_tiles = (EdgeTile*)(a0 + o_ftiles); db->t_offset = (int32_t*)(a0 + o_toff);
+    db->t_col = ta.out_col; db->t_row = ta.out_row; db->t_dist = ta.out_dist; db->t_weight = ta.out_weight;
   }
   db->ring = (float*)(a0 + o_ring); db->cgcnn = (float*)(a0 + o_cg); db->c0 = (float*)(a0 + o_c0);
   db->geom = (float*)(a0 + o_geom); db->gd = (float*)(a0 + o_gd);
@@ -427,11 +462,12 @@
 extern "C" {
 
 int scann_batch_upload(scann_handle_t* h, const scann_batch_t* b, scann_dbatch_t** out) { return upload_impl(h, b, out, false); }
-
-int scann_upload_padded(scann_handle_t* h, int32_t B, int32_t M, int32_t N, const int32_t* atomic, const void* atom_mask,
-                        int32_t atom_mask_size, const int32_t* neighbors, const void* neighbor_mask, int32_t neighbor_mask_size,
-                        const float* neighbor_weight, const float* neighbor_distance, scann_dbatch_t** out, int32_t* n_atom_out,
-                        int32_t* n_edge_out) {
+int scann_batch_upload_once(scann_handle_t* h, const scann_batch_t* b, scann_dbatch_t** out) { return upload_impl(h, b, out, false, nullptr, true); }
+
+static int upload_padded(scann_handle_t* h, int32_t B, int32_t M, int32_t N, const int32_t* atomic, const void* atom_mask,
+                         int32_t atom_mask_size, const int32_t* neighbors, const void* neighbor_mask, int32_t neighbor_mask_size,
+                         const float* neighbor_weight, const float* neighbor_distance, scann_dbatch_t** out, int32_t* n_atom_out,
+                         int32_t* n_edge_out, bool plan_fill) {
   if (!h || !out || B <= 0 || M <= 0 || N < 0 || !atomic || !atom_mask || (N > 0 && (!neighbors || !neighbor_mask || !neighbor_weight || !neighbor_distance)))
     return fail(h, SCANN_ERR_INVALID, "scann_upload_padded: bad argument");
   *out = nullptr;
@@ -443,11 +479,27 @@
   scann_batch_t pb{};
   pb.n_struct = B; pb.n_atom = na; pb.n_edge = ne; pb.mol_offset = mol.data(); pb.edge_offset = eoff.data();
   const PaddedSrc src{M, N, atomic, neighbors, neighbor_mask, neighbor_mask_size, neighbor_weight, neighbor_distance, row_of.data()};
-  const int r = upload_impl(h, &pb, out, false, &src);
+  const int r = upload_impl(h, &pb, out, false, &src, plan_fill);
   if (r) return r;
   if (n_atom_out) *n_atom_out = na;
   if (n_edge_out) *n_edge_out = ne;
   return SCANN_OK;
+}
+
+int scann_upload_padded(scann_handle_t* h, int32_t B, int32_t M, int32_t N, const int32_t* atomic, const void* atom_mask,
+                        int32_t atom_mask_size, const int32_t* neighbors, const void* neighbor_mask, int32_t neighbor_mask_size,
+                        const float* neighbor_weight, const float* neighbor_distance, scann_dbatch_t** out, int32_t* n_atom_out,
+                        int32_t* n_edge_out) {
+  return upload_padded(h, B, M, N, atomic, atom_mask, atom_mask_size, neighbors, neighbor_mask, neighbor_mask_size, neighbor_weight,
+                       neighbor_distance, out, n_atom_out, n_edge_out, false);
+}
+
+int scann_upload_padded_once(scann_handle_t* h, int32_t B, int32_t M, int32_t N, const int32_t* atomic, const void* atom_mask,
+                             int32_t atom_mask_size, const int32_t* neighbors, const void* neighbor_mask, int32_t neighbor_mask_size,
+                             const float* neighbor_weight, const float* neighbor_distance, scann_dbatch_t** out, int32_t* n_atom_out,
+                             int32_t* n_edge_out) {
+  return upload_padded(h, B, M, N, atomic, atom_mask, atom_mask_size, neighbors, neighbor_mask, neighbor_mask_size, neighbor_weight,
+                       neighbor_distance, out, n_atom_out, n_edge_out, true);
 }
 
 void scann_batch_free(scann_handle_t* h, scann_dbatch_t* db) {
diff --git a/scann--material_amd/csrc/scann_internal.h b/scann--material_amd/csrc/scann_internal.h
--- a/scann--material_amd/csrc/scann_internal.h
+++ b/scann--material_amd/csrc/scann_internal.h
@@ -359,9 +359,11 @@
                int tile_rows_req, int tile_atoms, bool allow_chunks, std::vector<EdgeTile>& tiles, std::vector<int32_t>& tile_part,
                std::vector<int32_t>& big_tab, std::vector<int32_t>& edge_row, int* tile_rows_out, int32_t* max_degree,
                int32_t* n_slot, std::string& err, bool fill_edge_row = true);
+constexpr int32_t PLAN_CHUNK = 128;
+constexpr int32_t PLAN_CHUNKS_PER_THREAD = 16;
 bool plan_tiles_filled(const int32_t* mol_offset, int32_t B, const int32_t* edge_offset, int32_t A, int rows, int tile_atoms,
                        const std::vector<EdgeTile>& contiguous, int32_t n_big, std::vector<int32_t>& atom_row,
-                       std::vector<int32_t>& tile_offset, std::vector<EdgeTile>& tiles);
+                       std::vector<int32_t>& tile_offset, std::vector<EdgeTile>& tiles, int32_t chunk = 0, int n_threads = 0);
 struct TileOrderArgs {
   const EdgeTile* tiles;
   int32_t n_tile, n_atom;
diff --git a/scann--material_amd/csrc/scann_pack.cpp b/scann--material_amd/csrc/scann_pack.cpp
--- a/scann--material_amd/csrc/scann_pack.cpp
+++ b/scann--material_amd/csrc/scann_pack.cpp
@@ -126,9 +126,71 @@
   return SCANN_OK;
 }
 
+static bool fill_chunk(const int32_t* mol_offset, int32_t s0, int32_t s1, const int32_t* edge_offset, int rows, int tile_atoms,
+                       int32_t* out_row, int32_t* out_off, std::vector<EdgeTile>& tiles) {
+  std::vector<int32_t> order_buf;
+  int32_t cnt[66] = {}, head[66], tail[66], fill[66];
+  int32_t k = mol_offset[s0], e = edge_offset[k];
+  EdgeTile cur{k, k, e, e};
+  for (int s = s0; s < s1; ++s) {
+    const int32_t a0 = mol_offset[s], a1 = mol_offset[s + 1];
+    int maxd = 0;
+    for (int a = a0; a < a1; ++a) {
+      const int d = edge_offset[a + 1] - edge_offset[a];
+      if (d > rows) return false;
+      ++cnt[d];
+      maxd = std::max(maxd, d);
+    }
+    uint64_t lo = 0;
+    bool top = false;
+    for (int d = 0, pos = 0; d <= maxd; ++d) {
+      head[d] = fill[d] = pos;
+      if (cnt[d]) { if (d < 64) lo |= 1ull << d; else top = true; }
+      pos += cnt[d];
+      tail[d] = pos;
+      cnt[d] = 0;
+    }
+    if (order_buf.size() < (size_t)(a1 - a0)) order_buf.resize((size_t)(a1 - a0) * 2);
+    int32_t* const order = order_buf.data();
+    for (int a = a0; a < a1; ++a) order[fill[edge_offset[a + 1] - edge_offset[a]]++] = a;
+    for (int left = a1 - a0; left > 0; --left) {
+      const int room = (k - cur.atom_begin) >= tile_atoms ? -1 : rows - (e - cur.edge_begin);
+      int d = -1;
+      if (room >= 64 && top) d = 64;
+      else if (room >= 0) {
+        const uint64_t fit = room >= 63 ? lo : lo & ((2ull << room) - 1);
+        if (fit) d = 63 - __builtin_clzll(fit);
+      }
+      if (d < 0) {
+        cur.atom_end = k; cur.edge_end = e;
+        tiles.push_back(cur);
+        cur = EdgeTile{k, k, e, e};
+        d = top ? 64 : 63 - __builtin_clzll(lo);
+      }
+      const int32_t a = order[head[d]++];
+      if (head[d] == tail[d]) { if (d < 64) lo &= ~(1ull << d); else top = false; }
+      out_row[k++] = a;
+      e += d;
+      out_off[k] = e;
+    }
+  }
+  cur.atom_end = k; cur.edge_end = e;
+  tiles.push_back(cur);
+  return true;
+}
+
+static int plan_threads(int32_t n_chunk, int n_threads) {
+  if (n_threads <= 0) {
+    const unsigned hw = std::thread::hardware_concurrency();
+    n_threads = (int)std::min<int64_t>(std::min<unsigned>(hw ? hw : 1u, 8u), n_chunk / PLAN_CHUNKS_PER_THREAD);
+    if (const char* e = getenv("SCANN_PLAN_THREADS")) n_threads = std::max(1, std::min(64, atoi(e)));
+  }
+  return std::max(1, std::min<int>(n_threads, n_chunk));
+}
+
 bool plan_tiles_filled(const int32_t* mol_offset, int32_t B, const int32_t* edge_offset, int32_t A, int rows, int tile_atoms,
                        const std::vector<EdgeTile>& contiguous, int32_t n_big, std::vector<int32_t>& atom_row,
-                       std::vector<int32_t>& tile_offset, std::vector<EdgeTile>& tiles) {
+                       std::vector<int32_t>& tile_offset, std::vector<EdgeTile>& tiles, int32_t chunk, int n_threads) {
   const auto identity = [&]() {
     atom_row.resize((size_t)A);
     for (int a = 0; a < A; ++a) atom_row[(size_t)a] = a;
@@ -139,64 +201,68 @@
   if (n_big > 0 || rows > 64 || rows <= 0 || tile_atoms <= 0 || contiguous.size() <= 1) return identity();
   atom_row.resize((size_t)A);
   tile_offset.resize((size_t)A + 1);
+  tile_offset[0] = 0;
   tiles.clear();
-  tiles.reserve(contiguous.size());
-  int32_t* const out_row = atom_row.data();
-  int32_t* const out_off = tile_offset.data();
-  out_off[0] = 0;
-  std::vector<int32_t> order_buf;
-  int32_t cnt[66] = {}, head[66], tail[66], fill[66];
-  EdgeTile cur{0, 0, 0, 0};
-  int32_t k = 0, e = 0;
-  for (int s = 0; s < B; ++s) {
-    const int32_t a0 = mol_offset[s], a1 = mol_offset[s + 1];
-    int maxd = 0;
-    for (int a = a0; a < a1; ++a) {
-      const int d = edge_offset[a + 1] - edge_offset[a];
-      if (d > rows) return identity();
-      ++cnt[d];
-      maxd = std::max(maxd, d);
-    }
-    uint64_t lo = 0;
-    bool top = false;
-    for (int d = 0, pos = 0; d <= maxd; ++d) {
-      head[d] = fill[d] = pos;
-      if (cnt[d]) { if (d < 64) lo |= 1ull << d; else top = true; }
-      pos += cnt[d];
-      tail[d] = pos;
-      cnt[d] = 0;
-    }
-    if (order_buf.size() < (size_t)(a1 - a0)) order_buf.resize((size_t)(a1 - a0) * 2);
-    int32_t* const order = order_buf.data();
-    for (int a = a0; a < a1; ++a) order[fill[edge_offset[a + 1] - edge_offset[a]]++] = a;
-    for (int left = a1 - a0; left > 0; --left) {
-      const int room = (k - cur.atom_begin) >= tile_atoms ? -1 : rows - (e - cur.edge_begin);
-      int d = -1;
-      if (room >= 64 && top) d = 64;
-      else if (room >= 0) {
-        const uint64_t fit = room >= 63 ? lo : lo & ((2ull << room) - 1);
-        if (fit) d = 63 - __builtin_clzll(fit);
-      }
-      if (d < 0) {
-        cur.atom_end = k; cur.edge_end = e;
-        tiles.push_back(cur);
-        cur = EdgeTile{k, k, e, e};
-        d = top ? 64 : 63 - __builtin_clzll(lo);
-      }
-      const int32_t a = order[head[d]++];
-      if (head[d] == tail[d]) { if (d < 64) lo &= ~(1ull << d); else top = false; }
-      out_row[k++] = a;
-      e += d;
-      out_off[k] = e;
-    }
-  }
-  cur.atom_end = k; cur.edge_end = e;
-  tiles.push_back(cur);
+  if (chunk <= 0 || chunk > B) chunk = B;
+  const int32_t n_chunk = (B + chunk - 1) / chunk;
+  if (n_chunk == 1) {
+    tiles.reserve(contiguous.size());
+    if (!fill_chunk(mol_offset, 0, B, edge_offset, rows, tile_atoms, atom_row.data(), tile_offset.data(), tiles)) return identity();
+  } else {
+    std::vector<std::vector<EdgeTile>> part((size_t)n_chunk);
+    std::vector<char> ok((size_t)n_chunk, 1);
+    const int n_thr = plan_threads(n_chunk, n_threads);
+    fan_out(n_thr, [&](int t) {
+      for (int32_t c = t; c < n_chunk; c += n_thr) {
+        part[(size_t)c].reserve((size_t)chunk * 4);
+        ok[(size_t)c] = fill_chunk(mol_offset, c * chunk, std::min(B, (c + 1) * chunk), edge_offset, rows, tile_atoms, atom_row.data(),
+                                   tile_offset.data(), part[(size_t)c]);
+      }
+    });
+    size_t n = 0;
+    for (int32_t c = 0; c < n_chunk; ++c) {
+      if (!ok[(size_t)c]) return identity();
+      n += part[(size_t)c].size();
+    }
+    tiles.reserve(n);
+    for (const std::vector<EdgeTile>& p : part) tiles.insert(tiles.end(), p.begin(), p.end());
+  }
   if (tiles.size() >= contiguous.size()) return identity();
   return true;
 }
 
 
+}
+
+static int plan_filled_abi(const char* who, const scann_batch_t* b, int32_t tile_rows, int32_t tile_atoms, int32_t chunk, int32_t n_threads,
+                           int32_t cap, int32_t* atom_row_out, int32_t* tile_offset_out, int32_t* tiles_out, int32_t* n_tiles) {
+  if (!b || !n_tiles || !atom_row_out || !tile_offset_out || !tiles_out || !b->mol_offset || !b->edge_offset || b->n_struct <= 0 ||
+      b->n_atom <= 0 || b->n_edge < 0 || (tile_rows != 32 && tile_rows != 64) || tile_atoms <= 0 || tile_atoms > 32)
+    return pack_fail((std::string(who) + ": bad argument").c_str());
+  if (b->mol_offset[0] != 0 || b->mol_offset[b->n_struct] != b->n_atom || b->edge_offset[0] != 0 || b->edge_offset[b->n_atom] != b->n_edge)
+    return pack_fail((std::string(who) + ": offsets do not cover the batch").c_str());
+  for (int s = 0; s < b->n_struct; ++s)
+    if (b->mol_offset[s + 1] <= b->mol_offset[s]) return pack_fail((std::string(who) + ": structure without atoms").c_str());
+  std::vector<scann::EdgeTile> contiguous, tiles;
+  std::vector<int32_t> part, big, row, atom_row, tile_offset;
+  int rows = 0;
+  int32_t maxdeg = 0, nslot = 0;
+  std::string err;
+  const int r = scann::plan_tiles(b->mol_offset, b->n_struct, b->edge_offset, nullptr, b->n_atom, b->n_edge, tile_rows, tile_atoms, true,
+                                  contiguous, part, big, row, &rows, &maxdeg, &nslot, err, false);
+  if (r) {
+    t_pack_error = std::string(who) + ": " + err;
+    return r;
+  }
+  const bool filled = scann::plan_tiles_filled(b->mol_offset, b->n_struct, b->edge_offset, b->n_atom, rows, tile_atoms, contiguous,
+                                               (int32_t)big.size() / 3, atom_row, tile_offset, tiles,
+                                               chunk < 0 ? 0 : chunk ? chunk : scann::PLAN_CHUNK, n_threads);
+  *n_tiles = (int32_t)tiles.size();
+  if ((int32_t)tiles.size() > cap) return pack_fail((std::string(who) + ": output capacity too small").c_str());
+  memcpy(atom_row_out, atom_row.data(), atom_row.size() * 4);
+  memcpy(tile_offset_out, tile_offset.data(), tile_offset.size() * 4);
+  memcpy(tiles_out, tiles.data(), tiles.size() * sizeof(scann::EdgeTile));
+  return filled ? 1 : 0;
 }
 
 extern "C" {
@@ -459,32 +525,14 @@
 
 int scann_plan_tiles_filled(const scann_batch_t* b, int32_t tile_rows, int32_t tile_atoms, int32_t cap, int32_t* atom_row_out,
                             int32_t* tile_offset_out, int32_t* tiles_out, int32_t* n_tiles) {
-  if (!b || !n_tiles || !atom_row_out || !tile_offset_out || !tiles_out || !b->mol_offset || !b->edge_offset || b->n_struct <= 0 ||
-      b->n_atom <= 0 || b->n_edge < 0 || (tile_rows != 32 && tile_rows != 64) || tile_atoms <= 0 || tile_atoms > 32)
-    return pack_fail("scann_plan_tiles_filled: bad argument");
-  if (b->mol_offset[0] != 0 || b->mol_offset[b->n_struct] != b->n_atom || b->edge_offset[0] != 0 || b->edge_offset[b->n_atom] != b->n_edge)
-    return pack_fail("scann_plan_tiles_filled: offsets do not cover the batch");
-  for (int s = 0; s < b->n_struct; ++s)
-    if (b->mol_offset[s + 1] <= b->mol_offset[s]) return pack_fail("scann_plan_tiles_filled: structure without atoms");
-  std::vector<scann::EdgeTile> contiguous, tiles;
-  std::vector<int32_t> part, big, row, atom_row, tile_offset;
-  int rows = 0;
-  int32_t maxdeg = 0, nslot = 0;
-  std::string err;
-  const int r = scann::plan_tiles(b->mol_offset, b->n_struct, b->edge_offset, nullptr, b->n_atom, b->n_edge, tile_rows, tile_atoms, true,
-                                  contiguous, part, big, row, &rows, &maxdeg, &nslot, err, false);
-  if (r) {
-    t_pack_error = "scann_plan_tiles_filled: " + err;
-    return r;
-  }
-  const bool filled = scann::plan_tiles_filled(b->mol_offset, b->n_struct, b->edge_offset, b->n_atom, rows, tile_atoms, contiguous,
-                                               (int32_t)big.size() / 3, atom_row, tile_offset, tiles);
-  *n_tiles = (int32_t)tiles.size();
-  if ((int32_t)tiles.size() > cap) return pack_fail("scann_plan_tiles_filled: output capacity too small");
-  memcpy(atom_row_out, atom_row.data(), atom_row.size() * 4);
-  memcpy(tile_offset_out, tile_offset.data(), tile_offset.size() * 4);
-  memcpy(tiles_out, tiles.data(), tiles.size() * sizeof(scann::EdgeTile));
-  return filled ? 1 : 0;
-}
-
-}
+  return plan_filled_abi("scann_plan_tiles_filled", b, tile_rows, tile_atoms, -1, 0, cap, atom_row_out, tile_offset_out, tiles_out, n_tiles);
+}
+
+int scann_plan_tiles_chunked(const scann_batch_t* b, int32_t tile_rows, int32_t tile_atoms, int32_t chunk, int32_t n_threads, int32_t cap,
+                             int32_t* atom_row_out, int32_t* tile_offset_out, int32_t* tiles_out, int32_t* n_tiles) {
+  if (chunk < 0 || n_threads < 0) return pack_fail("scann_plan_tiles_chunked: bad argument");
+  return plan_filled_abi("scann_plan_tiles_chunked", b, tile_rows, tile_atoms, chunk, n_threads, cap, atom_row_out, tile_offset_out,
+                         tiles_out, n_tiles);
+}
+
+}
diff --git a/scann--material_amd/csrc/scann_runtime.cpp b/scann--material_amd/csrc/scann_runtime.cpp
--- a/scann--material_amd/csrc/scann_runtime.cpp
+++ b/scann--material_amd/csrc/scann_runtime.cpp
@@ -405,6 +405,7 @@
   if (const char* ar = getenv("SCANN_ATOM_ROWS")) h->atom_rows = atoi(ar);
   if (const char* fb = getenv("SCANN_FUSE_BASIS")) h->fuse_basis = atoi(fb) != 0;
   if (const char* tf = getenv("SCANN_TILE_FILL")) h->tile_fill = atoi(tf) != 0;
+  if (const char* pu = getenv("SCANN_PLAN_AT_UPLOAD")) h->plan_at_upload = atoi(pu) != 0;
   if (const char* st = getenv("SCANN_SPECIES_TABLES")) h->species_tables = atoi(st) != 0;
   if (const char* sg = getenv("SCANN_STRICT_RANGE")) h->strict_range = atoi(sg) != 0;
   if (const char* fe = getenv("SCANN_EXACT")) h->force_exact = atoi(fe) != 0;
diff --git a/scann--material_amd/csrc/scann_runtime.h b/scann--material_amd/csrc/scann_runtime.h
--- a/scann--material_amd/csrc/scann_runtime.h
+++ b/scann--material_amd/csrc/scann_runtime.h
@@ -115,6 +115,7 @@
   int atom_rows = 0;
   int fuse_basis = 1;
   int tile_fill = 1;
+  int plan_at_upload = -1;
   int species_tables = 1;
   bool generic = false;
   float* g_weights = nullptr;
diff --git a/scann--material_amd/scann/_hip.py b/scann--material_amd/scann/_hip.py
--- a/scann--material_amd/scann/_hip.py
+++ b/scann--material_amd/scann/_hip.py
@@ -97,6 +97,7 @@
     ("scann_slice_batch", C.c_int, [_P] * 8 + [C.c_int32, C.c_int64] + [_P] * 7),
     ("scann_plan_tiles", C.c_int, [C.POINTER(Batch), C.c_int32, C.c_int32, C.c_int32, C.c_int32, _P, _P, C.POINTER(C.c_int32), C.POINTER(C.c_int32)]),
     ("scann_plan_tiles_filled", C.c_int, [C.POINTER(Batch), C.c_int32, C.c_int32, C.c_int32, _P, _P, _P, C.POINTER(C.c_int32)]),
+    ("scann_plan_tiles_chunked", C.c_int, [C.POINTER(Batch), C.c_int32, C.c_int32, C.c_int32, C.c_int32, C.c_int32, _P, _P, _P, C.POINTER(C.c_int32)]),
     ("scann_batch_tile_plan", C.c_int, [_P, _P, _P]),
     ("scann_exact_reruns", C.c_int64, [_P]),
     ("scann_weights_exact", C.c_int, [_P]),
@@ -105,6 +106,9 @@
     ("scann_count_padded", C.c_int, [C.c_int32, C.c_int32, C.c_int32, _P, C.c_int32, _P, C.c_int32, _P, _P, _P, C.POINTER(C.c_int32), C.POINTER(C.c_int32)]),
     ("scann_upload_padded", C.c_int, [_P, C.c_int32, C.c_int32, C.c_int32, _P, _P, C.c_int32, _P, _P, C.c_int32, _P, _P, C.POINTER(_P),
                                       C.POINTER(C.c_int32), C.POINTER(C.c_int32)]),
+    ("scann_batch_upload_once", C.c_int, [_P, C.POINTER(Batch), C.POINTER(_P)]),
+    ("scann_upload_padded_once", C.c_int, [_P, C.c_int32, C.c_int32, C.c_int32, _P, _P, C.c_int32, _P, _P, C.c_int32, _P, _P, C.POINTER(_P),
+                                           C.POINTER(C.c_int32), C.POINTER(C.c_int32)]),
     ("scann_batch_read_csr", C.c_int, [_P, _P, _P, _P, _P, _P, _P, _P]),
     ("scann_host_copy", C.c_int, [_P, _P, C.c_int64]),
     ("scann_set_outputs", C.c_int, [_P, C.c_uint64, C.c_int32]),
@@ -1181,7 +1185,8 @@
     _check_runtime_env()
     lib = C.CDLL(p)
     for name, res, args in SYMBOLS:
-        if name in ("scann_plan_tiles_filled", "scann_batch_tile_plan", "scann_weights_exact") and os.environ.get("SCANN_HIP_LIB") and not hasattr(lib, name):
+        if name in ("scann_plan_tiles_filled", "scann_batch_tile_plan", "scann_weights_exact", "scann_plan_tiles_chunked", "scann_batch_upload_once",
+                    "scann_upload_padded_once") and os.environ.get("SCANN_HIP_LIB") and not hasattr(lib, name):
             continue
         fn = getattr(lib, name)
         fn.restype = res
@@ -1346,14 +1351,18 @@
     return rc, tiles[:nt.value].copy(), part[:nt.value].copy(), ns.value
 
 
-def plan_tiles_filled(packed, tile_rows=64, tile_atoms=24):
+def plan_tiles_filled(packed, tile_rows=64, tile_atoms=24, chunk=None, threads=0):
     lib = load_library()
     cap = packed.n_atom + packed.n_edge // 32 + 2
     atom_row, tile_offset = np.empty(packed.n_atom, np.int32), np.empty(packed.n_atom + 1, np.int32)
     tiles = np.empty((cap, 4), np.int32)
     nt = C.c_int32(0)
     st = packed.as_struct()
-    rc = lib.scann_plan_tiles_filled(C.byref(st), tile_rows, tile_atoms, cap, _ptr(atom_row), _ptr(tile_offset), _ptr(tiles), C.byref(nt))
+    if chunk is None:
+        rc = lib.scann_plan_tiles_filled(C.byref(st), tile_rows, tile_atoms, cap, _ptr(atom_row), _ptr(tile_offset), _ptr(tiles), C.byref(nt))
+    else:
+        rc = lib.scann_plan_tiles_chunked(C.byref(st), tile_rows, tile_atoms, int(chunk), int(threads), cap, _ptr(atom_row), _ptr(tile_offset),
+                                          _ptr(tiles), C.byref(nt))
     if rc < 0:
         raise ScannHipError(rc, (lib.scann_pack_last_error() or b"").decode())
     return bool(rc), atom_row, tile_offset, tiles[:nt.value].copy()
@@ -1608,13 +1617,22 @@
                                                   _ptr(wgt), _ptr(dst), _ptr(y), _ptr(ga)))
         return y, ga
 
-    def upload(self, packed):
+    def _upload_fn(self, name, once):
+        return getattr(self.lib, name + "_once" if once and hasattr(self.lib, name + "_once") else name)
+
+    def upload(self, packed, once=False):
         st = packed.as_struct()
         db = _P()
-        self._check(self.lib.scann_batch_upload(self._h, C.byref(st), C.byref(db)))
+        self._check(self._upload_fn("scann_batch_upload", once)(self._h, C.byref(st), C.byref(db)))
         return ResidentBatch(self, packed, db)
 
-    def upload_padded(self, inputs):
+    def upload_once(self, packed):
+        return self.upload(packed, once=True)
+
+    def upload_padded_once(self, inputs):
+        return self.upload_padded(inputs, once=True)
+
+    def upload_padded(self, inputs, once=False):
         atomic = np.ascontiguousarray(inputs["atomic"], dtype=np.int32)
         B, M = atomic.shape
         amask, asz = _mask_arg(np.asarray(inputs["atom_mask"]).reshape(B, M))
@@ -1626,8 +1644,8 @@
         if nbr.shape != (B, M, N) or nmask.shape != nbr.shape or wgt.shape != nbr.shape or dst.shape != nbr.shape or amask.shape != (B, M):
             raise ValueError("inconsistent input shapes")
         db, na, ne = _P(), C.c_int32(0), C.c_int32(0)
-        self._check(self.lib.scann_upload_padded(self._h, B, M, N, _ptr(atomic), _ptr(amask), asz, _ptr(nbr), _ptr(nmask), nsz, _ptr(wgt),
-                                                 _ptr(dst), C.byref(db), C.byref(na), C.byref(ne)))
+        self._check(self._upload_fn("scann_upload_padded", once)(self._h, B, M, N, _ptr(atomic), _ptr(amask), asz, _ptr(nbr), _ptr(nmask), nsz,
+                                                                 _ptr(wgt), _ptr(dst), C.byref(db), C.byref(na), C.byref(ne)))
         return ResidentBatch(self, PaddedInfo(B, na.value, ne.value, amask != 0 if amask.dtype != np.bool_ else amask), db)
 
     def read_csr(self, rb):
diff --git a/scann--material_amd/scann/models/scann_model.py b/scann--material_amd/scann/models/scann_model.py
--- a/scann--material_amd/scann/models/scann_model.py
+++ b/scann--material_amd/scann/models/scann_model.py
@@ -815,11 +815,14 @@
         finally:
             index.free()
 
-    def _upload_padded(self, inputs):
+    def _upload_padded(self, inputs, once=False):
         m, eng = self.config["model"], self.engine
         if m["feature"] == "atomic" and not m["use_ring"] and not eng.training:
-            return eng.upload_padded(inputs)
-        return eng.upload(_hip.pack_inputs(inputs))
+            return (self._once("upload_padded") if once else eng.upload_padded)(inputs)
+        return (self._once("upload") if once else eng.upload)(_hip.pack_inputs(inputs))
+
+    def _once(self, name):
+        return getattr(self.engine, name + "_once", None) or getattr(self.engine, name)
 
     def _read_outputs(self, rb, sel):
         eng, out = self.engine, {}
@@ -882,7 +885,7 @@
             if want_ga:
                 gas.append(ga)
 
-        self._pipeline(((functools.partial(self._upload_padded, {key: v[i:i + C] for key, v in inputs.items()}), i)
+        self._pipeline(((functools.partial(self._upload_padded, {key: v[i:i + C] for key, v in inputs.items()}, once=True), i)
                         for i in range(0, B, C)), finish, sel)
         y = np.concatenate(ys).reshape(-1, 1)
         if not want_ga and sel is None:
@@ -913,6 +916,7 @@
         per_struct = {n: [] for n in sel[0]} if sel is not None else None
         n = len(dataset)
         grouped = getattr(dataset, "batches", None)
+        upload = self._once("upload")
 
         def jobs():
             for g0 in range(0, n, group):
@@ -930,7 +934,7 @@
                         tg.append(np.asarray(tgt, dtype=np.float32))
                     pk = _hip.concat_packed(parts) if len(parts) > 1 else parts[0]
                     counts = [p.n_struct for p in parts]
-                yield functools.partial(eng.upload, pk), (tg, pk, counts)
+                yield functools.partial(upload, pk), (tg, pk, counts)
 
         def finish(rb, tag):
             tg, pk, counts = tag
```

Result: no change. 1.957 million, median of 2 (-0.1%).
